# NOAA-GFDL/icebergs

Measured on AMD Instinct MI355X. Metric: berg_steps_per_sec, higher is better.
Workload: dtype f64; 1 GPU; BASELINE configs[4] per-GPU share with configs[1] physics: 10000000 synthetic bergs/GPU (random mass classes), 360x200 lat-lon ocean grid, RK4 drag+Coriolis+melt+mass spreading, dt=1800 s, ignore_traj=T; bergs_per_gpu=10000000, grid=360x200, exchange=none (1 GPU), bergs_alive_at_end=9999583

## Files before the change

### icebergs_amd/csrc/kid_handle.hpp

```cpp
#pragma once
#include "kid_mem.hpp"

struct HipAllocator {
  static constexpr int unknown_error = (int)hipErrorInvalidValue;
  const hipStream_t *stream;
  int alloc(void **p, size_t bytes, kid::MemKind k) const { return (int)(k == kid::MEM_PINNED ? hipHostMalloc(p, bytes) : hipMalloc(p, bytes)); }
  int release(void *p, kid::MemKind k) const { return (int)(k == kid::MEM_PINNED ? hipHostFree(p) : hipFree(p)); }
  int fill(void *p, int byte, size_t bytes) const { return (int)hipMemsetAsync(p, byte, bytes, *stream); }
  int copy(void *dst, const void *src, size_t bytes) const { return (int)hipMemcpy(dst, src, bytes, hipMemcpyDeviceToDevice); }
};
struct Scratch { void *p = nullptr; size_t bytes = 0; };
struct HipMem : kid::MemOwner<HipAllocator> {
  explicit HipMem(const hipStream_t *stream) : kid::MemOwner<HipAllocator>(HipAllocator{stream}) {}
  template <class T> hipError_t dev(T *&p, size_t count, int fill = kid::MEM_NOFILL, kid::MemKind k = kid::MEM_DEVICE) { void *q = nullptr; const int e = alloc(&q, count * sizeof(T), k, fill); p = (T *)q; return (hipError_t)e; }
  template <class T> hipError_t pinned(T *&p, size_t count) { return dev(p, count, kid::MEM_NOFILL, kid::MEM_PINNED); }
  template <class T> hipError_t drop(T *&p) { void *q = p; const int e = release(&q); p = (T *)q; return (hipError_t)e; }
  template <class T> hipError_t regrow(T *&p, size_t keep_count, size_t count) { void *q = p; const int e = grow(&q, keep_count * sizeof(T), count * sizeof(T)); p = (T *)q; return (hipError_t)e; }
  hipError_t reserve(Scratch &t, size_t bytes) {
    if (t.p && t.bytes >= bytes) return hipSuccess;
    int e = release(&t.p);
    if (!e) e = alloc(&t.p, bytes, kid::MEM_DEVICE);
    t.bytes = e ? 0 : bytes;
    return (hipError_t)e;
  }
};

namespace {
enum { KID_PERM_MAX = KID_NB_F64 + KID_NB_I32 + 2 };
struct PermTable { const void *src[KID_PERM_MAX]; void *dst[KID_PERM_MAX]; int n8, n4; };
}

struct ForcingSet { VelRec *vel = nullptr; TrcRec *trc = nullptr; double *pkt = nullptr; DevGrid *d_grid = nullptr; };
struct ForcingState {
  bool have_static = false, have_forcing = false;
  bool have_centres = false;
  bool have_planes = false;
  bool held[KID_NFORCING] = {};
};

struct kid_handle {
  int device = 0;
  hipStream_t own_stream = nullptr, stream = nullptr;
  HipMem mem{&stream}, rp_mem{&stream};
  kid_grid_desc gd{};
  kid_params params{};
  int ni = 0, nj = 0;
  size_t ncell = 0;
  int64_t capacity = 0, n = 0;
  double auto_growth = 0.; int64_t auto_min_free = 0, auto_max_capacity = 0;
  double *d_static[KID_NGRID_STATIC] = {}, *d_forcing[KID_NFORCING] = {};
  GeoRec *d_geo = nullptr; double *d_hotok = nullptr; double *d_latref = nullptr;
  double *d_acc_own = nullptr, *d_acc = nullptr;
  double *d_out = nullptr;
  double *d_totals = nullptr;
  BergPtrs bp{};
  BergPtrs *d_bp = nullptr;
  kid_params *d_params = nullptr;
  bool tables_dirty = true;
  Scratch scan_tmp;
  unsigned long long *d_count = nullptr;
  int *d_redo_list = nullptr;
  hipStream_t side_stream = nullptr; bool pipelined = false;
  int *d_redo_list2 = nullptr, *d_redo_count2 = nullptr;
  int *d_redo_cnt[2][2] = {{nullptr, nullptr}, {nullptr, nullptr}};
  int redo_parity = 0; bool redo_prezeroed = false, acc_prezeroed = false;
  kid::ZeroState zs;
  unsigned long long hot_zero_mask = 0ull;
  bool tail_valid = false;
  bool mig_mode = false;
  int32_t *d_keep = nullptr;
  long long mig_last[2] = {0, 0};
  long long halo_last[2] = {0, 0};
  bool halo_rows_live = false;
  bool env_ever_stored = false;
  bool env_off_requested = false;
  double *d_orient = nullptr;
  hipEvent_t evF[2] = {nullptr, nullptr}, evG[2] = {nullptr, nullptr}; bool evG_live[2] = {false, false};
  int side_mode = 0; int *d_lane = nullptr, *d_lane_alt = nullptr; hipEvent_t evR = nullptr; int lane_step = 1; bool lanes_active = false, carry_valid = false, evC_live = false;
  hipEvent_t evC = nullptr, evP = nullptr;
  ForcingSet fset[2]; int forc_parity = 0;
  struct DebugOpts { bool stable_resort = false, no_plain_build = false, fl_unfused = false, new_order_unfused = false, mts_always_label = false, mts_no_fused = false, rebin_eager = false, chksum_timing = false, no_zero_skip = false;
                     int mts_fused_blocks_cap = 0, mts_poll_limit = 0; } dbg;
  int32_t *d_iceberg_counter = nullptr;
  bool fl_place_warm = false;
  unsigned fl_step = 0;
  int *d_fl_cursor = nullptr;
  int *d_fl_promoted = nullptr;
  int32_t *d_fl_head = nullptr, *d_fl_next = nullptr; int64_t *d_fl_newid = nullptr; long long fl_ev_capacity = 0;
  unsigned *d_key[2] = {nullptr, nullptr}, *d_idx[2] = {nullptr, nullptr};
  Scratch sort_tmp;
  BergPtrs bp_alt{};
  bool rebin_pending = false;
  int64_t rebin_fused_count = 0;
  struct RebinPlan { PermTable t{}; int moved_f[KID_NB_F64] = {}; int nmf = 0; unsigned long long moved = 0ull, zero_skipped = 0ull; const unsigned *perm = nullptr; long long n = 0; } rplan;
  RebinTab *d_rb = nullptr;
  unsigned *d_cell_hist = nullptr; Scratch cscan_tmp; bool stable_resort = false;
  int resort_interval = 16, steps_since_sort = 0;
  MtsDev mts{}; MtsDev *d_mts = nullptr;
  int mb = 0; bool mts_ready = false, mts_dirty = true, have_bonds = false, visited = false;
  unsigned long long *d_key64[2] = {nullptr, nullptr}; int *d_rows[2] = {nullptr, nullptr};
  int *d_static_rows = nullptr; long long static_rows_n = -1, static_rows_cap = 0;
  unsigned long long *d_last_key = nullptr; int *d_order_flag = nullptr; long long order_n = -1;
  unsigned long long *d_bond_sig = nullptr; bool labels_stale = true;
  MtsDev mts_shadow{}; bool mts_shadow_valid = false;
  int conglom_batch = 8;
  Scratch mts_tmp;
  unsigned long long *d_bond_words = nullptr;
  double bond_ext[2] = {0., 0.}; bool bond_ext_valid = false;
  hipGraphExec_t sub_graph_exec = nullptr;
  long long sub_graph_n = -1; int sub_graph_steps = 0; bool sub_graph_pair = false; double sub_graph_dt = 0.; hipStream_t sub_graph_stream = nullptr;
  bool use_graph = true;
  int fused_blocks[2] = {0, 0};
  bool fused_ran = false;
  Flags flags{0, 0, 1, 0, 0};
  bool traj_on = false; kid_traj_params traj_params{}; double *d_traj_f[64] = {}; double *d_traj_day = nullptr; int64_t *d_traj_id = nullptr;
  int32_t *d_traj_year = nullptr, *d_traj_nbonds = nullptr; unsigned long long *d_traj_cursor = nullptr; long long traj_capacity = 0, traj_count_bound = 0; int traj_nf = 0;
  double *d_mig_buf = nullptr; long long mig_capacity = 0; unsigned long long *mig_word = nullptr;
  double *halo_buf = nullptr; long long halo_capacity = 0;
  double *d_btraj_f[16] = {}; int64_t *d_btraj_id[2] = {}; int32_t *d_btraj_i[2] = {}; long long btraj_capacity = 0, btraj_count_bound = 0;
  double *d_spread_mass_old = nullptr;
  double *d_spread_mass_old_own = nullptr;
  ForcingState forc;
  int restart_locate = 0;
  double *d_calv_state = nullptr, *d_calv_scal = nullptr, *d_calv_part = nullptr; unsigned char *d_calv_flag = nullptr; int2 *d_calv_list = nullptr; double *calv_host = nullptr; kid_calving_params calv_params{};
  bool calving_on = false, calving_first_call = true, rmean_init = false, rmean_hflx_init = false;
  double *d_ingest_stage = nullptr; size_t ingest_stage_count = 0; unsigned long long *d_ingest_key = nullptr;
  bool profile = false;
  hipEvent_t ev0 = nullptr, ev1 = nullptr, ev2 = nullptr, ev3 = nullptr;
  std::vector<std::pair<hipEvent_t, hipEvent_t>> pending;
  double berg_ms = 0., all_ms = 0.; int64_t berg_launches = 0;
  bool repro = false;
  struct Repro { double *stage = nullptr; int32_t *key = nullptr; unsigned long long *mask = nullptr; int *srows = nullptr; long long srows_n = -1;
                 unsigned long long *k64[2] = {nullptr, nullptr}; int *rows[2] = {nullptr, nullptr}; unsigned *k32[2] = {nullptr, nullptr};
                 int *cs = nullptr; double *cell_heat = nullptr, *part = nullptr; Scratch tmp; } rp;
  double *d_budget = nullptr, *d_budget_plane = nullptr;
  std::string err;
};

#define KID_HIP(h, call)                                                                      \
  do {                                                                                        \
    hipError_t e__ = (call);                                                                  \
    if (e__ != hipSuccess) {                                                                  \
      (h)->err = std::string(#call) + ": " + hipGetErrorString(e__);                          \
      return KID_EHIP;                                                                        \
    }                                                                                         \
  } while (0)

extern "C" {
static int refresh_tables(kid_handle *h), join_side(kid_handle *h);
static int rebin_flush(kid_handle *h);
static int rebin_plan(kid_handle *h, bool dead_last);
static int rebin_core(kid_handle *h, bool with_lane, int *list, const int *list_count), rebin_apply(kid_handle *h, bool with_lane, int *list, const int *list_count);
static bool plain_namelist(const kid_handle *h), lanes_eligible(const kid_handle *h);
static int repro_refuse(kid_handle *h);
static int mts_check_timeout(kid_handle *h), mts_fold_scalars(kid_handle *h);
static int halo_bergs_supported(kid_handle *h, const char *what);
static int auto_reserve(kid_handle *h, int64_t need, const char *what);
}
```

### icebergs_amd/csrc/kid_hip.hip

```cpp
#include <algorithm>
#include <chrono>
#include <cmath>
#include <cstdio>
#include <cstdlib>
#include <cstring>
#include <string.h>
#include <string>
#include <type_traits>
#include <utility>
#include <vector>
#include <unordered_map>
#include <hip/hip_runtime.h>
#include <rocprim/rocprim.hpp>
#include "../../include/kid.h"
#include "kid_device.hpp"
#include "kid_thermo.hpp"
#include "kid_footloose.hpp"
#include "kid_berg_kernel.hpp"
#include "kid_rows_plan.hpp"
#include "kid_fl_contact.hpp"
#include "kid_reserve_plan.hpp"

using namespace kid;

#ifdef KID_HOT_PLAIN_SEPARATE
namespace kid { void launch_hot_plain(bool store_env, bool rebin, unsigned nblocks, void *stream, const DevGrid *gtab, const kid_params *pp, const void *bp, long long n,
                                      double *acc, size_t ncell, const void *flags, const void *redo); }
#else
#include "kid_hot_plain.inc"
#endif

namespace {

__global__ void __launch_bounds__(256) footloose_kernel(const DevGrid g, const kid_params *__restrict__ pp, const BergPtrs *__restrict__ bt,
                                                        const FlChildCtx cx, double *__restrict__ acc, const size_t ncell) {
  const long long q = (long long)blockIdx.x * 256ll + threadIdx.x;
  if (q >= cx.n) return;
  const BergPtrs &b = *bt;
  if (b.i[KID_BI_ALIVE][q] == 0) return;
  footloose_one(g, *pp, b, cx, q, acc, ncell, acc - KID_NSCALAR);
}

__global__ void set_berg_table_kernel(const BergPtrs src, BergPtrs *dst) { if (threadIdx.x == 0 && blockIdx.x == 0) *dst = src; }
__global__ void set_rebin_table_kernel(const RebinTab src, RebinTab *dst) { if (threadIdx.x == 0 && blockIdx.x == 0) *dst = src; }
__global__ void set_params_kernel(const kid_params src, kid_params *dst) { if (threadIdx.x == 0 && blockIdx.x == 0) *dst = src; }
__global__ void set_time_kernel(int32_t year, double yearday, kid_params *dst) { if (threadIdx.x == 0 && blockIdx.x == 0) { dst->current_year = year; dst->current_yearday = yearday; } }

#include "kid_mts.inc"
#include "kid_fl_interact.inc"

}

#include "kid_handle.hpp"

static int halo_rows_refuse(kid_handle *h, const char *what) {
  if (!h->halo_rows_live) return KID_OK;
  h->err = std::string(what) + ": halo rows are resident (copies of the neighbours' bergs, kid_unpack_immigrants); the next kid_evolve_icebergs retires them";
  return KID_EINVAL;
}
#include "kid_cells.inc"

static int check_params(kid_handle *h, const kid_params *p) {
  if (p->dem && !p->mts) { h->err = "dem needs mts=T (the DEM forces live on the MTS sub-steps)"; return KID_EINVAL; }
  if (p->mts) {
    if (p->Runge_not_Verlet) { h->err = "Runge_not_Verlet must be false to use MTS or DEM (FW:1485-1490)"; return KID_EINVAL; }
    if (p->old_interp_flds_order) { h->err = "old_interp_flds_order is false whenever mts/dem is on (FW:1483)"; return KID_EINVAL; }
    if (p->mts_sub_steps < 1) { h->err = "mts_sub_steps must be >= 1 (pass the value ice_bergs_framework_init derives, FW:1296-1301)"; return KID_EINVAL; }
    if (p->dem && !p->explicit_inner_mts) { h->err = "dem forces explicit_inner_mts=T (FW:1433)"; return KID_EINVAL; }
    if (p->dem && !p->iceberg_bonds_on) { h->err = "dem needs iceberg_bonds_on"; return KID_EINVAL; }
    if (p->max_bonds < 1 || p->max_bonds > KID_MAX_BONDS) { h->err = "max_bonds out of range"; return KID_EINVAL; }
    if (p->use_broken_bonds_for_substep_contact && !(p->break_bonds_on_sub_steps && p->dem && p->iceberg_bonds_on)) {
      h->err = "use_broken_bonds_for_substep_contact requires break_bonds_on_sub_steps, dem and iceberg_bonds_on (FW:1438-1447)"; return KID_EINVAL; }
    if (p->footloose) { h->err = "footloose together with mts is not implemented"; return KID_EUNSUPPORTED; }
  } else if (p->interactive_icebergs_on || p->iceberg_bonds_on) {
    if (p->Runge_not_Verlet) { h->err = "interacting / bonded bergs under the single-time-step scheme are implemented for Verlet only (Runge_not_Verlet=F)"; return KID_EUNSUPPORTED; }
    if (p->footloose && p->iceberg_bonds_on) { h->err = "footloose together with iceberg_bonds_on: bonded footloose calving (edge elements that calve, IB:2566-2585) is not implemented"; return KID_EUNSUPPORTED; }
    if (p->iceberg_bonds_on && !p->interactive_icebergs_on) { h->err = "iceberg_bonds_on without interactive_icebergs_on is not implemented"; return KID_EUNSUPPORTED; }
    if (p->max_bonds < 1 || p->max_bonds > KID_MAX_BONDS) { h->err = "max_bonds out of range"; return KID_EINVAL; }
  }
  if (p->tidal_drift > 0.) { h->err = "tidal_drift needs FMS's random stream: not supported"; return KID_EUNSUPPORTED; }
  if (p->find_melt_using_spread_mass && (p->mts || p->interactive_icebergs_on || p->footloose)) {
    h->err = "find_melt_using_spread_mass is implemented for the plain evolve loop only (no bonds, interactions or footloose)";
    return KID_EUNSUPPORTED;
  }
  if (p->Runge_not_Verlet && p->footloose) { h->err = "Runge_not_Verlet must be false to use footloose (FW:1485-1490)"; return KID_EINVAL; }
  if (p->footloose && !p->use_operator_splitting) { h->err = "use_operator_splitting must be true to use footloose (FW:1476)"; return KID_EINVAL; }
  return KID_OK;
}

extern "C" {

#ifndef KID_BUILD_ID
#define KID_BUILD_ID "unknown"
#endif
const char *kid_version(void) {
  return "kid_hip 0.3 (gfx950) src " KID_BUILD_ID
#ifdef KID_EXACT_MATH
         " exact-math"
#endif
#ifdef KID_EXPERIMENTS
         " EXPERIMENTS"
#endif
      ;
}
int64_t kid_sizeof(int which) {
  switch (which) { case 0: return (int64_t)sizeof(kid_params); case 1: return (int64_t)sizeof(kid_grid_desc);
                   case 2: return (int64_t)sizeof(kid_berg_soa); case 3: return (int64_t)sizeof(kid_bond_soa);
                   case 4: return (int64_t)sizeof(kid_forcing_in);
                   case 5: return (int64_t)sizeof(kid_calving_params); case 6: return (int64_t)sizeof(kid_calving_in); default: return -1; }
}
#ifdef KID_EXP_TIMING
int kid_exp_timing(unsigned long long *out, int reset) {
  if (out) {
    std::vector<unsigned long long> all((size_t)KID_TPROF_WAVES * 16);
    if (hipMemcpyFromSymbol(all.data(), HIP_SYMBOL(kid_tprof), all.size() * sizeof(unsigned long long)) != hipSuccess) return KID_EHIP;
    for (int q = 0; q < 16; ++q) out[q] = 0ull;
    for (size_t r = 0; r < (size_t)KID_TPROF_WAVES; ++r) for (int q = 0; q < 16; ++q) out[q] += all[r * 16 + q];
  }
  if (reset) {
    void *sym = nullptr;
    if (hipGetSymbolAddress(&sym, HIP_SYMBOL(kid_tprof)) != hipSuccess || hipMemset(sym, 0, (size_t)KID_TPROF_WAVES * 16 * sizeof(unsigned long long)) != hipSuccess) return KID_EHIP;
  }
  return KID_OK;
}
#endif
static thread_local std::string destroy_err;
const char *kid_last_error(const kid_handle *h) { return h ? h->err.c_str() : destroy_err.empty() ? "null handle" : destroy_err.c_str(); }

int kid_create(const kid_grid_desc *grid, const kid_params *params, int64_t capacity, int device, kid_handle **out) {
  if (!grid || !params || !out || capacity <= 0) return KID_EINVAL;
  if (capacity > (int64_t(1) << 29)) return KID_EINVAL;
  int ndev = 0;
  if (hipGetDeviceCount(&ndev) != hipSuccess || ndev <= 0) return KID_ENODEV;
  if (device < 0 || device >= ndev) return KID_ENODEV;
  kid_handle *h = new kid_handle();
  *out = h;
  h->device = device;
  KID_HIP(h, hipSetDevice(device));
  h->gd = *grid;
  h->ni = grid->ied - grid->isd + 1; h->nj = grid->jed - grid->jsd + 1;
  if (h->ni < 5 || h->nj < 5 || grid->isc - grid->isd < 2 || grid->ied - grid->iec < 2 || grid->jsc - grid->jsd < 2 || grid->jed - grid->jec < 2) {
    h->err = "grid needs a halo of at least 2 cells"; return KID_EINVAL;
  }
  h->ncell = (size_t)h->ni * (size_t)h->nj;
  int rc = check_params(h, params);
  if (rc) return rc;
  h->params = *params;
  h->flags.footprint = footprint_needed(h->params) ? 1 : 0;
  h->capacity = capacity;
  if (getenv("KID_MTS_NO_GRAPH")) h->use_graph = false;
  h->dbg.stable_resort = getenv("KID_STABLE_RESORT") != nullptr; h->dbg.no_plain_build = getenv("KID_NO_PLAIN_BUILD") != nullptr;
  h->dbg.fl_unfused = getenv("KID_FL_UNFUSED") != nullptr; h->dbg.new_order_unfused = getenv("KID_NEW_ORDER_UNFUSED") != nullptr;
  h->dbg.rebin_eager = getenv("KID_REBIN_EAGER") != nullptr; h->dbg.chksum_timing = getenv("KID_CHKSUM_TIMING") != nullptr;
  h->dbg.no_zero_skip = getenv("KID_NO_ZERO_SKIP") != nullptr;
  h->dbg.mts_always_label = getenv("KID_MTS_ALWAYS_LABEL") != nullptr; h->dbg.mts_no_fused = getenv("KID_MTS_NO_FUSED") != nullptr;
  if (const char *e = getenv("KID_MTS_FUSED_BLOCKS_CAP")) h->dbg.mts_fused_blocks_cap = atoi(e);
  if (const char *e = getenv("KID_MTS_POLL_LIMIT")) h->dbg.mts_poll_limit = atoi(e);
  KID_HIP(h, hipStreamCreateWithFlags(&h->own_stream, hipStreamNonBlocking));
  h->stream = h->own_stream;
  const size_t cap = (size_t)capacity;
  for (auto &plane : h->d_static) KID_HIP(h, h->mem.dev(plane, h->ncell, 0));
  for (auto &plane : h->d_forcing) KID_HIP(h, h->mem.dev(plane, h->ncell, 0));
  for (ForcingSet &fs : h->fset) {
    KID_HIP(h, h->mem.dev(fs.vel, h->ncell)); KID_HIP(h, h->mem.dev(fs.trc, h->ncell)); KID_HIP(h, h->mem.dev(fs.d_grid, 1));
    KID_HIP(h, h->mem.dev(fs.pkt, h->ncell * PK_GSTRIDE, 0));
  }
  KID_HIP(h, h->mem.dev(h->d_geo, h->ncell));
  KID_HIP(h, h->mem.dev(h->d_hotok, h->ncell, 0));
  if (grid->grid_is_latlon) KID_HIP(h, h->mem.dev(h->d_latref, 2 * h->ncell));
  KID_HIP(h, h->mem.dev(h->d_acc_own, (size_t)KID_NACC * h->ncell + KID_NSCALAR, 0));
  h->d_acc = h->d_acc_own + KID_NSCALAR;
  KID_HIP(h, h->mem.dev(h->d_out, (size_t)KID_NOUT * h->ncell, 0));
  KID_HIP(h, h->mem.dev(h->d_totals, KID_NSCALAR, 0));
  for (auto &field : h->bp.f) KID_HIP(h, h->mem.dev(field, cap, 0));
  for (auto &field : h->bp.i) KID_HIP(h, h->mem.dev(field, cap, 0));
  KID_HIP(h, h->mem.dev(h->bp.id, cap, 0));
  KID_HIP(h, h->mem.dev(h->d_bp, 1));
  KID_HIP(h, h->mem.dev(h->d_rb, 1));
  KID_HIP(h, h->mem.dev(h->d_params, 1));
  KID_HIP(h, h->mem.dev(h->d_lane, cap, 0));
  KID_HIP(h, h->mem.dev(h->d_count, 4));
  KID_HIP(h, h->mem.dev(h->d_iceberg_counter, h->ncell, 0));
  KID_HIP(h, h->mem.dev(h->d_fl_cursor, 1));
  for (int **q : {&h->d_redo_list, &h->d_redo_list2}) KID_HIP(h, h->mem.dev(*q, cap));
  KID_HIP(h, h->mem.dev(h->d_redo_count2, 4, 0));
  for (int part = 0; part < 2; ++part) for (int par = 0; par < 2; ++par) h->d_redo_cnt[part][par] = h->d_redo_count2 + (2 * part + par);
  for (hipEvent_t *e : {&h->evC, &h->evP, &h->evF[0], &h->evF[1], &h->evG[0], &h->evG[1]}) KID_HIP(h, hipEventCreateWithFlags(e, hipEventDisableTiming));
  for (hipEvent_t *e : {&h->ev0, &h->ev1, &h->ev2, &h->ev3}) KID_HIP(h, hipEventCreate(e));
  KID_HIP(h, hipStreamSynchronize(h->stream));
  return KID_OK;
}

int kid_destroy(kid_handle *h) {
  if (!h) return KID_EINVAL;
  (void)hipSetDevice(h->device);
  (void)hipDeviceSynchronize();
  if (h->sub_graph_exec) (void)hipGraphExecDestroy(h->sub_graph_exec);
  for (hipEvent_t e : {h->evR, h->evC, h->evP, h->evF[0], h->evF[1], h->evG[0], h->evG[1], h->ev0, h->ev1, h->ev2, h->ev3}) if (e) (void)hipEventDestroy(e);
  for (auto &pe : h->pending) { (void)hipEventDestroy(pe.first); (void)hipEventDestroy(pe.second); }
  if (h->own_stream) (void)hipStreamDestroy(h->own_stream);
  const int e_rp = h->rp_mem.free_all(), e_mem = h->mem.free_all();
  const hipError_t e = (hipError_t)(e_rp ? e_rp : e_mem);
  delete h;
  if (e == hipSuccess) return KID_OK;
  destroy_err = std::string("kid_destroy: freeing the handle's memory: ") + hipGetErrorString(e);
  return KID_EHIP;
}

int kid_memory_in_use(int64_t *device_bytes, int64_t *pinned_bytes) {
  if (device_bytes) *device_bytes = kid::mem_in_use(kid::MEM_DEVICE).load();
  if (pinned_bytes) *pinned_bytes = kid::mem_in_use(kid::MEM_PINNED).load();
  return KID_OK;
}

int kid_set_params(kid_handle *h, const kid_params *params) {
  if (!h || !params) return KID_EINVAL;
  int rc = check_params(h, params);
  if (rc) return rc;
  if (!h->tables_dirty && h->d_params) {
    kid_params a = h->params, b = *params;
    a.current_year = b.current_year = 0; a.current_yearday = b.current_yearday = 0.;
    if (std::memcmp(&a, &b, sizeof(kid_params)) == 0) {
      h->params = *params;
      KID_HIP(h, hipSetDevice(h->device));
      hipLaunchKernelGGL(set_time_kernel, dim3(1), dim3(64), 0, h->stream, params->current_year, params->current_yearday, h->d_params);
      KID_HIP(h, hipGetLastError());
      return KID_OK;
    }
  }
  h->params = *params;
  h->tables_dirty = true;
  h->labels_stale = true;
  h->flags.footprint = footprint_needed(h->params) ? 1 : 0;
  if (!h->params.old_interp_flds_order && !h->env_off_requested) h->flags.store_env = 1;
  return KID_OK;
}
static int join_side(kid_handle *h) {
  for (int q = 0; q < 2; ++q)
    if (h->evG_live[q]) { KID_HIP(h, hipStreamWaitEvent(h->stream, h->evG[q], 0)); }
  if (h->evC_live) { KID_HIP(h, hipStreamWaitEvent(h->stream, h->evC, 0)); }
  return KID_OK;
}
static int lanes_drain(kid_handle *h) {
  const int rc = join_side(h);
  if (rc || !h->lanes_active) return rc;
  KID_HIP(h, hipMemsetAsync(h->d_lane, 0, (size_t)h->capacity * sizeof(int), h->stream));
  if (h->d_lane_alt) KID_HIP(h, hipMemsetAsync(h->d_lane_alt, 0, (size_t)h->capacity * sizeof(int), h->stream));
  h->lanes_active = false; h->carry_valid = false; h->lane_step = 1;
  return KID_OK;
}
int kid_set_side_stream(kid_handle *h, void *s, int enable) {
  if (!h) return KID_EINVAL;
  KID_HIP(h, hipSetDevice(h->device));
  int rc = join_side(h);
  if (rc) return rc;
  KID_HIP(h, hipStreamSynchronize(h->stream));
  { const int rc_d = lanes_drain(h); if (rc_d) return rc_d; }
  { const int rc_f = rebin_flush(h); if (rc_f) return rc_f; }
  KID_HIP(h, hipStreamSynchronize(h->stream));
  h->evG_live[0] = h->evG_live[1] = false; h->evC_live = false;
  h->side_stream = (hipStream_t)s;
  h->pipelined = enable == 1;
  h->side_mode = (s && enable == 2) ? 2 : 0;
  return KID_OK;
}
int kid_set_stream(kid_handle *h, void *s) {
  if (!h) return KID_EINVAL;
  h->stream = (hipStream_t)s;
  return KID_OK;
}
static inline int id_iNg(const kid_grid_desc &d) { return d.gni > 0 ? d.gni : d.iec - d.isc + 1; }
static inline int id_ij0(const kid_grid_desc &d) { return d.gni > 0 ? d.gi0 + d.gni * d.gj0 : 0; }
int kid_sync(kid_handle *h) {
  if (!h) return KID_EINVAL;
  KID_HIP(h, hipSetDevice(h->device));
  { const int rc_j = join_side(h); if (rc_j) return rc_j; }
  KID_HIP(h, hipStreamSynchronize(h->stream));
  return mts_check_timeout(h);
}

#include "kid_ingest.inc"
}
#include "kid_rows.inc"
extern "C" {

int kid_upload_bergs(kid_handle *h, const kid_berg_soa *host) {
  if (!h || !host || host->n < 0) return KID_EINVAL;
  if (host->n > h->capacity) { const int rc = auto_reserve(h, host->n, "kid_upload_bergs"); if (rc) return rc; }
  if (host->n > h->capacity) { h->err = "more bergs than capacity"; return KID_ECAPACITY; }
  { const int rc = rows_enter(h, ROWS_CHANGE); if (rc) return rc; }
  const size_t n = (size_t)host->n;
  for (int f = 0; f < KID_NB_F64; ++f) {
    if (host->f64[f]) KID_HIP(h, hipMemcpyAsync(h->bp.f[f], host->f64[f], n * sizeof(double), hipMemcpyHostToDevice, h->stream));
    else KID_HIP(h, hipMemsetAsync(h->bp.f[f], 0, n * sizeof(double), h->stream));
  }
  for (int f = 0; f < KID_NB_I32; ++f) {
    if (host->i32[f]) KID_HIP(h, hipMemcpyAsync(h->bp.i[f], host->i32[f], n * sizeof(int32_t), hipMemcpyHostToDevice, h->stream));
    else if (f == KID_BI_ALIVE) { if (n) hipLaunchKernelGGL(fill_i32_kernel, dim3((unsigned)((n + 255) / 256)), dim3(256), 0, h->stream, h->bp.i[f], 1, (long long)n); }
    else KID_HIP(h, hipMemsetAsync(h->bp.i[f], 0, n * sizeof(int32_t), h->stream));
  }
  if (host->id) KID_HIP(h, hipMemcpyAsync(h->bp.id, host->id, n * sizeof(int64_t), hipMemcpyHostToDevice, h->stream));
  else KID_HIP(h, hipMemsetAsync(h->bp.id, 0, n * sizeof(int64_t), h->stream));
  if (host->i32[KID_BI_INE] && host->i32[KID_BI_JNE]) {
    for (size_t k = 0; k < n; ++k) {
      const int i = host->i32[KID_BI_INE][k], j = host->i32[KID_BI_JNE][k];
      if (i < h->gd.isc - 1 || i > h->gd.iec + 1 || j < h->gd.jsc - 1 || j > h->gd.jec + 1) {
        h->err = "berg cell index (ine,jne) outside the computational domain"; return KID_EINVAL;
      }
    }
  } else if (n > 0) { h->err = "ine/jne are required"; return KID_EINVAL; }
  if (h->bp.orient) { h->bp.orient = nullptr; h->tables_dirty = true; }
  rows_replaced(h, host);
  h->visited = false; h->have_bonds = false;
  KID_HIP(h, hipStreamSynchronize(h->stream));
  return KID_OK;
}

int kid_download_bergs(kid_handle *h, kid_berg_soa *host) {
  if (!h || !host) return KID_EINVAL;
  if (host->n < h->n) { h->err = "host SoA too small"; return KID_EINVAL; }
  { const int rc = rows_enter(h, ROWS_READ); if (rc) return rc; }
  const size_t n = (size_t)h->n;
  for (int f = 0; f < KID_NB_F64; ++f)
    if (host->f64[f]) KID_HIP(h, hipMemcpyAsync(host->f64[f], h->bp.f[f], n * sizeof(double), hipMemcpyDeviceToHost, h->stream));
  for (int f = 0; f < KID_NB_I32; ++f)
    if (host->i32[f]) KID_HIP(h, hipMemcpyAsync(host->i32[f], h->bp.i[f], n * sizeof(int32_t), hipMemcpyDeviceToHost, h->stream));
  if (host->id) KID_HIP(h, hipMemcpyAsync(host->id, h->bp.id, n * sizeof(int64_t), hipMemcpyDeviceToHost, h->stream));
  KID_HIP(h, hipStreamSynchronize(h->stream));
  host->n = h->n;
  return KID_OK;
}

int kid_set_store_environment(kid_handle *h, int on) {
  if (!h) return KID_EINVAL;
  h->flags.store_env = on ? 1 : 0;
  h->env_off_requested = !on;
  return KID_OK;
}

static int refresh_tables(kid_handle *h) {
  if (h->tables_dirty) {
    const int rc = join_side(h);
    if (rc) return rc;
    hipLaunchKernelGGL(set_berg_table_kernel, dim3(1), dim3(64), 0, h->stream, h->bp, h->d_bp);
    hipLaunchKernelGGL(set_params_kernel, dim3(1), dim3(64), 0, h->stream, h->params, h->d_params);
    for (int par = 0; par < 2; ++par) hipLaunchKernelGGL(set_grid_kernel, dim3(1), dim3(64), 0, h->stream, dev_grid(h, par), h->fset[par].d_grid);
    KID_HIP(h, hipGetLastError());
    h->tables_dirty = false;
  }
  return KID_OK;
}
static int fl_place_children(kid_handle *h, long long n_old, int m, unsigned step) {
  if (!h->fl_place_warm) {
    h->fl_place_warm = true;
    hipLaunchKernelGGL(fl_place_children_kernel<BergPtrs>, dim3(1), dim3(64), 0, h->stream, dev_grid(h), (const kid_params *)h->d_params, (const BergPtrs *)h->d_bp, n_old, 0, step);
    KID_HIP(h, hipGetLastError());
  }
  if (m <= 0) return KID_OK;
  hipLaunchKernelGGL(fl_place_children_kernel<BergPtrs>, dim3((unsigned)((m + 63) / 64)), dim3(64), 0, h->stream, dev_grid(h), (const kid_params *)h->d_params, (const BergPtrs *)h->d_bp, n_old, m, step);
  KID_HIP(h, hipGetLastError());
  return KID_OK;
}
static int fl_assign_ids(kid_handle *h, long long n_old, int m) {
  if (m <= 0) return KID_OK;
  if (!h->d_fl_head) KID_HIP(h, h->mem.dev(h->d_fl_head, h->ncell, 0xff));
  if (m > h->fl_ev_capacity) {
    KID_HIP(h, h->mem.drop(h->d_fl_next));
    KID_HIP(h, h->mem.drop(h->d_fl_newid));
    h->fl_ev_capacity = std::max<long long>(2ll * m, 4096);
    KID_HIP(h, h->mem.dev(h->d_fl_next, (size_t)h->fl_ev_capacity));
    KID_HIP(h, h->mem.dev(h->d_fl_newid, (size_t)h->fl_ev_capacity));
  }
  const FlIdCtx x{h->d_fl_head, h->d_fl_next, h->d_fl_newid, h->d_iceberg_counter, n_old, m, id_iNg(h->gd), id_ij0(h->gd)};
  const dim3 grid((unsigned)((m + 255) / 256)), block(256);
  const DevGrid g = dev_grid(h);
  hipLaunchKernelGGL(fl_assign_ids_push<BergPtrs>, grid, block, 0, h->stream, g, (const BergPtrs *)h->d_bp, x);
  hipLaunchKernelGGL(fl_assign_ids_rank<BergPtrs>, grid, block, 0, h->stream, g, (const BergPtrs *)h->d_bp, x);
  hipLaunchKernelGGL(fl_assign_ids_store<BergPtrs>, grid, block, 0, h->stream, g, (const BergPtrs *)h->d_bp, x);
  KID_HIP(h, hipGetLastError());
  return KID_OK;
}
static const char *const fl_full = "footloose calving ran out of capacity: create the handle with room for child bergs";
int kid_footloose_calving(kid_handle *h) {
  if (!h) return KID_EINVAL;
  { const int rc_h = halo_rows_refuse(h, "kid_footloose_calving"); if (rc_h) return rc_h; }
  if (!h->params.footloose || h->n == 0) return KID_OK;
  KID_HIP(h, hipSetDevice(h->device));
  int rc = repro_refuse(h);
  if (rc) return rc;
  rc = rebin_flush(h);
  if (rc) return rc;
  rc = refresh_tables(h);
  if (rc) return rc;
  h->flags.has_fl = 1;
  h->zs.launched_other();
  rc = auto_reserve(h, h->n + h->auto_min_free, "kid_footloose_calving");
  if (rc) return rc;
  KID_HIP(h, hipMemsetAsync(h->d_fl_cursor, 0, sizeof(int), h->stream));
  const unsigned fl_step_now = h->fl_step;
  FlChildCtx cx{h->d_fl_cursor, h->d_iceberg_counter, (long long)h->n, (long long)h->capacity, h->gd.iec - h->gd.isc + 1, h->fl_step++};
  hipLaunchKernelGGL(footloose_kernel, dim3((unsigned)((h->n + 255) / 256)), dim3(256), 0, h->stream, dev_grid(h), h->d_params, h->d_bp, cx, h->d_acc, h->ncell);
  KID_HIP(h, hipGetLastError());
  int appended = 0;
  KID_HIP(h, hipMemcpyAsync(&appended, h->d_fl_cursor, sizeof(int), hipMemcpyDeviceToHost, h->stream));
  KID_HIP(h, hipStreamSynchronize(h->stream));
  if (appended <= h->capacity - h->n) {
    rc = fl_place_children(h, h->n, appended, fl_step_now);
    if (!rc) rc = fl_assign_ids(h, h->n, appended);
    if (rc) return rc;
  }
  return rows_appended(h, appended, nullptr, fl_full);
}
double kid_footloose_uniform(int32_t seed, int64_t berg_id, int64_t step, int32_t draw) {
  return kid_fl_uniform((uint32_t)seed, berg_id, (uint32_t)step, (uint32_t)draw);
}
int kid_set_footloose_step(kid_handle *h, int64_t step) {
  if (!h || step < 0) return KID_EINVAL;
  h->fl_step = (unsigned)step;
  return KID_OK;
}
int kid_get_footloose_step(kid_handle *h, int64_t *step) {
  if (!h || !step) return KID_EINVAL;
  *step = (int64_t)h->fl_step;
  return KID_OK;
}
int kid_set_iceberg_counter(kid_handle *h, const int32_t *counter) {
  if (!h || !counter) return KID_EINVAL;
  KID_HIP(h, hipSetDevice(h->device));
  KID_HIP(h, hipMemcpy(h->d_iceberg_counter, counter, h->ncell * sizeof(int32_t), hipMemcpyHostToDevice));
  return KID_OK;
}
int kid_get_iceberg_counter(kid_handle *h, int32_t *counter) {
  if (!h || !counter) return KID_EINVAL;
  KID_HIP(h, hipSetDevice(h->device));
  KID_HIP(h, hipStreamSynchronize(h->stream));
  KID_HIP(h, hipMemcpy(counter, h->d_iceberg_counter, h->ncell * sizeof(int32_t), hipMemcpyDeviceToHost));
  return KID_OK;
}

#include "kid_mts_host.inc"
#include "kid_calving.inc"
#include "kid_repro.inc"
}
#include "kid_bond_init.inc"
#include "kid_budget.inc"
#include "kid_launch.inc"
#include "kid_reserve.inc"
extern "C" {

int kid_last_redo_count(kid_handle *h, int64_t *count) {
  if (!h || !count) return KID_EINVAL;
  KID_HIP(h, hipSetDevice(h->device));
  { const int rc_j = join_side(h); if (rc_j) return rc_j; }
  int c[4] = {0, 0, 0, 0};
  KID_HIP(h, hipMemcpyAsync(c, h->d_redo_count2, 4 * sizeof(int), hipMemcpyDeviceToHost, h->stream));
  KID_HIP(h, hipStreamSynchronize(h->stream));
  *count = (int64_t)c[0 + h->redo_parity] + (h->pipelined ? (int64_t)c[2 + h->redo_parity] : 0);
  return KID_OK;
}
int kid_rebin_fused_count(kid_handle *h, int64_t *count) {
  if (!h || !count) return KID_EINVAL;
  *count = h->rebin_fused_count;
  return KID_OK;
}
int kid_hot_zero_mask(kid_handle *h, uint64_t *mask) {
  if (!h || !mask) return KID_EINVAL;
  *mask = (uint64_t)h->hot_zero_mask;
  return KID_OK;
}
int kid_profile_enable(kid_handle *h, int on) {
  if (!h) return KID_EINVAL;
  h->profile = on != 0;
  h->berg_ms = 0.; h->all_ms = 0.; h->berg_launches = 0;
  return KID_OK;
}
int kid_profile_get(kid_handle *h, double *berg_ms, int64_t *launches, double *all_ms) {
  if (!h) return KID_EINVAL;
  KID_HIP(h, hipSetDevice(h->device));
  KID_HIP(h, hipStreamSynchronize(h->stream));
  for (auto &pe : h->pending) {
    float ms = 0.f;
    KID_HIP(h, hipEventElapsedTime(&ms, pe.first, pe.second));
    h->berg_ms += ms;
    (void)hipEventDestroy(pe.first); (void)hipEventDestroy(pe.second);
  }
  h->pending.clear();
  if (berg_ms) *berg_ms = h->berg_ms;
  if (launches) *launches = h->berg_launches;
  if (all_ms) *all_ms = h->all_ms;
  return KID_OK;
}

}

#include "kid_locate.inc"
#include "kid_restart.inc"
#include "kid_traj.inc"
#include "kid_migrate.inc"
#include "kid_halo_bergs.inc"
#include "kid_halo.inc"
#include "kid_chksum.inc"
#include "kid_chksum_device.inc"
```

### icebergs_amd/csrc/kid_launch.inc

```

static bool plain_namelist(const kid_handle *h) {
  const kid_params &p = h->params;
  bool same = true;
#define KID_X(name, plain, flp) same = same && (p.name == (decltype(p.name))(plain));
  KID_SWITCHES(KID_X)
#undef KID_X
  const Flags &f = h->flags;
  return same && h->gd.grid_is_latlon && !p.pass_fields_to_ocean_model && !f.has_static && !f.has_fl && !f.footprint && !f.no_diag &&
         !h->dbg.no_plain_build;
}
static bool fl_profile_namelist(const kid_handle *h) {
  const kid_params &p = h->params;
  bool same = true;
#define KID_X(name, plain, flp) same = same && (p.name == (decltype(p.name))(flp));
  KID_SWITCHES(KID_X)
#undef KID_X
  const Flags &f = h->flags;
  return same && !h->gd.grid_is_latlon && !p.pass_fields_to_ocean_model && !f.has_static && f.has_fl && !f.footprint && !f.no_diag && !h->dbg.no_plain_build;
}
static bool lanes_eligible(const kid_handle *h) {
  const kid_params &p = h->params;
  return kid::lanes_eligible(h->side_mode, h->side_stream != nullptr, h->repro, p.static_icebergs != 0, p.mts != 0, p.interactive_icebergs_on != 0,
                             p.footloose != 0, p.grounding_fraction, p.find_melt_using_spread_mass != 0, (long long)h->n);
}

struct BergLaunch { const DevGrid *gtab; bool plain, flprof; };
static BergLaunch berg_launch(const kid_handle *h) { return {h->fset[h->forc_parity].d_grid, plain_namelist(h), fl_profile_namelist(h)}; }

template <bool RK, bool OLD, unsigned PH, bool FAST, int K, bool STAGE>
static int launch_instance(kid_handle *h, const BergLaunch &c, hipStream_t s, unsigned nblocks, const Redo &redo) {
  static_assert(instance_exists(OLD, PH, STAGE), "no call site requests this instance (kid_launch_select.hpp)");
  hipLaunchKernelGGL((berg_kernel<RK, OLD, PH, FAST, K, STAGE>), dim3(nblocks), dim3(FAST ? KID_HOT_WG : 64), 0, s, c.gtab, h->d_params, h->d_bp, (long long)h->n, h->d_acc, h->ncell, h->flags, redo);
  KID_HIP(h, hipGetLastError());
  return KID_OK;
}
template <bool RK, bool OLD, unsigned PH, bool STAGE>
static int launch_hot(kid_handle *h, const BergLaunch &c, hipStream_t s, const Redo &redo, bool rebin = false) {
  const unsigned nbp = (unsigned)((redo.klen + KID_HOT_WG - 1) / KID_HOT_WG);
  const int k = hot_build_k(RK, OLD, PH, c.plain, c.flprof, h->flags.store_env != 0, STAGE);
  h->hot_zero_mask = 0ull;
  if constexpr (hot_build_k(RK, OLD, PH, true, false, false, STAGE) == 1) {
    if (k == 1 || k == 3) {
      Redo plain = redo;
      plain.zero = h->hot_zero_mask = known_zero_mask(h);
      kid::launch_hot_plain(k == 3, rebin, nbp, (void *)s, c.gtab, h->d_params, h->d_bp, (long long)h->n, h->d_acc, h->ncell, &h->flags, &plain);
      KID_HIP(h, hipGetLastError());
      return KID_OK;
    }
  }
  if constexpr (hot_build_k(RK, OLD, PH, false, true, false, STAGE) == 2) {
    if (k == 2 && !rebin) return launch_instance<RK, OLD, PH, true, 2, STAGE>(h, c, s, nbp, redo);
  }
  if (rebin || k != 0) { h->err = "no such hot build of the per-berg kernel"; return KID_EINVAL; }
  return launch_instance<RK, OLD, PH, true, 0, STAGE>(h, c, s, nbp, redo);
}
template <bool RK, bool OLD, unsigned PH, bool STAGE>
static int launch_general(kid_handle *h, const BergLaunch &c, hipStream_t s, const Redo &redo, long long rows) {
  return launch_instance<RK, OLD, PH, false, 0, STAGE>(h, c, s, (unsigned)std::min<long long>((rows + 63) / 64, 2048), redo);
}
template <unsigned PH, class F>
static int with_instance(kid_handle *h, bool stage, F &&f) {
  const bool rk = h->params.Runge_not_Verlet != 0, old = h->params.old_interp_flds_order != 0;
  auto go = [&](auto RK, auto OLD, auto STAGE) -> int {
    if constexpr (instance_exists(decltype(OLD)::value, PH, decltype(STAGE)::value)) return f(RK, OLD, STAGE);
    else { h->err = "no per-berg kernel for this phase mask, interpolation order and summation mode"; return KID_EINVAL; }
  };
  auto order = [&](auto RK, auto STAGE) { return old ? go(RK, std::true_type{}, STAGE) : go(RK, std::false_type{}, STAGE); };
  auto integrator = [&](auto STAGE) { return rk ? order(std::true_type{}, STAGE) : order(std::false_type{}, STAGE); };
  return stage ? integrator(std::true_type{}) : integrator(std::false_type{});
}

static int wait_general_builds(kid_handle *h, int part, int nparts) {
  if (h->evG_live[part]) KID_HIP(h, hipStreamWaitEvent(h->stream, h->evG[part], 0));
  if (nparts == 1 && h->evG_live[1]) KID_HIP(h, hipStreamWaitEvent(h->stream, h->evG[1], 0));
  return KID_OK;
}
static int zero_redo_counter(kid_handle *h, int *count) {
  if (!h->redo_prezeroed) KID_HIP(h, hipMemsetAsync(count, 0, sizeof(int), h->stream));
  return KID_OK;
}
struct ProfilePair { hipEvent_t e0 = nullptr, e1 = nullptr; };
static int profile_start(kid_handle *h, ProfilePair &t) {
  if (!h->profile) return KID_OK;
  KID_HIP(h, hipEventCreate(&t.e0)); KID_HIP(h, hipEventCreate(&t.e1));
  KID_HIP(h, hipEventRecord(t.e0, h->stream));
  return KID_OK;
}
static int profile_stop(kid_handle *h, const ProfilePair &t) {
  if (!h->profile) return KID_OK;
  KID_HIP(h, hipEventRecord(t.e1, h->stream));
  h->pending.emplace_back(t.e0, t.e1); h->berg_launches++;
  return KID_OK;
}
template <unsigned PH>
static int rebin_take_or_flush(kid_handle *h, bool whole, RebinTab &rtab, bool &fused) {
  fused = false;
  if (!h->rebin_pending) return KID_OK;
  fused = PH == PH_STEP && rebin_fusable(h) && whole && h->rplan.n == h->n && (h->rplan.zero_skipped & ~known_zero_mask(h)) == 0ull &&
          rebin_table(h, h->flags.store_env ? 3 : 1, rtab);
  return fused ? KID_OK : rebin_flush(h);
}
static int rebin_bind(kid_handle *h, const RebinTab &rtab, Redo &redo) {
  hipLaunchKernelGGL(set_rebin_table_kernel, dim3(1), dim3(64), 0, h->stream, rtab, h->d_rb);
  KID_HIP(h, hipGetLastError());
  redo.rb = h->d_rb; redo.perm = h->rplan.perm;
  return KID_OK;
}
static int rebin_hand_over(kid_handle *h, Redo &redo) {
  h->rebin_pending = false; redo.rb = nullptr; redo.perm = nullptr; h->rebin_fused_count++;
  return rebin_swap(h);
}
template <bool RK, bool OLD, unsigned PH>
static int launch_general_part(kid_handle *h, const BergLaunch &c, const Redo &redo, int part, int nparts) {
  hipStream_t gs = (nparts == 2) ? h->side_stream : h->stream;
  if (nparts == 2) { KID_HIP(h, hipEventRecord(h->evF[part], h->stream)); KID_HIP(h, hipStreamWaitEvent(gs, h->evF[part], 0)); }
  const int rc = launch_general<RK, OLD, PH, false>(h, c, gs, redo, redo.klen);
  if (rc) return rc;
  if (nparts == 2) KID_HIP(h, hipEventRecord(h->evG[part], gs));
  h->evG_live[part] = nparts == 2;
  return KID_OK;
}
template <unsigned PH>
static int launch_berg_part(kid_handle *h, const BergLaunch &c, bool stage, const RebinTab *rtab, Redo redo, int part, int nparts) {
  int rc = KID_OK;
  if (rtab) { rc = rebin_bind(h, *rtab, redo); if (rc) return rc; }
  rc = wait_general_builds(h, part, nparts);
  if (!rc) rc = zero_redo_counter(h, redo.count);
  ProfilePair t;
  if (!rc) rc = profile_start(h, t);
  if (rc) return rc;
  return with_instance<PH>(h, stage, [&](auto RK, auto OLD, auto STAGE) -> int {
    constexpr bool rk = decltype(RK)::value, old = decltype(OLD)::value;
    int r = launch_hot<rk, old, PH, decltype(STAGE)::value>(h, c, h->stream, redo, rtab != nullptr);
    if constexpr (decltype(STAGE)::value) {
      if (!r) r = launch_general<rk, old, PH, true>(h, c, h->stream, redo, redo.klen);
      if (!r) r = profile_stop(h, t);
      h->evG_live[part] = false;
      return r;
    } else {
      if (!r) r = profile_stop(h, t);
      if (!r && rtab) r = rebin_hand_over(h, redo);
      return r ? r : launch_general_part<rk, old, PH>(h, c, redo, part, nparts);
    }
  });
}
template <unsigned PH>
static int launch_phase(kid_handle *h, long long range_k0 = 0, long long range_len = -1) {
  if (need_forcing(h)) return KID_EINVAL;
  if (h->n == 0 || range_len == 0) return KID_OK;
  const bool old = h->params.old_interp_flds_order != 0, whole = range_k0 == 0 && range_len < 0;
  if (!old && !(PH & PH_INTERP) && (PH & (PH_EVOLVE | PH_THERMO)) && !h->flags.store_env) {
    h->err = "this entry point reads the bergs' stored environment, which kid_set_store_environment has switched off (use kid_run_step, or switch it on)";
    return KID_EINVAL;
  }
  h->zs.launched_berg((PH & PH_EVOLVE) != 0, (PH & PH_THERMO) != 0, h->params.Runge_not_Verlet != 0, h->params.bergy_bit_erosion_fraction == 0.,
                      h->flags.has_fl != 0, (PH & PH_FL) != 0);
  int rc = repro_refuse(h);
  if (!rc) rc = lanes_drain(h);
  RebinTab rtab;
  bool rebin_fused = false;
  if (!rc) rc = rebin_take_or_flush<PH>(h, whole, rtab, rebin_fused);
  if (!rc) rc = refresh_tables(h);
  if (rc) return rc;
  const BergLaunch c = berg_launch(h);
  rows_killed(h);
  if (h->flags.store_env || !old) h->env_ever_stored = true;
  const bool stage = (PH & PH_SCATTER) != 0 && h->repro;
  const int nparts = launch_parts(h->pipelined, stage, h->params.mts != 0, h->params.footloose != 0, (long long)h->n, range_len < 0);
  const long long half = ((h->n / 2 + 255) / 256) * 256;
  for (int part = 0; part < nparts && !rc; ++part) {
    const long long k0 = (nparts == 1) ? range_k0 : (part == 0 ? 0 : half);
    const long long klen = (nparts == 1) ? (range_len < 0 ? h->n : range_len) : (part == 0 ? half : h->n - half);
    const Redo redo{part == 0 ? h->d_redo_list : h->d_redo_list2, h->d_redo_cnt[part][h->redo_parity], k0, klen, nullptr, 0,
                    h->d_fl_cursor, h->d_iceberg_counter, (long long)h->capacity, h->gd.iec - h->gd.isc + 1, h->fl_step,
                    StageTab{h->rp.stage, h->rp.key, h->rp.mask, (long long)h->capacity}};
    rc = launch_berg_part<PH>(h, c, stage, rebin_fused ? &rtab : nullptr, redo, part, nparts);
  }
  if (nparts == 1) h->evG_live[1] = false;
  h->redo_prezeroed = false;
  if (rc) return rc;
  if (stage) return repro_fold(h, (PH & PH_THERMO) != 0, (PH & (PH_SPREAD | PH_TSPREAD)) != 0, range_k0, range_len < 0 ? h->n : range_len);
  return KID_OK;
}
template <unsigned PH>
static int launch_berg(kid_handle *h, long long range_k0 = 0, long long range_len = -1) {
  static_assert(instance_exists(true, PH, false) && instance_exists(false, PH, false), "this mask is bound to one order: launch_ordered");
  return launch_phase<PH>(h, range_k0, range_len);
}
template <unsigned X>
static int launch_ordered(kid_handle *h, long long range_k0 = 0, long long range_len = -1) {
  static_assert(!(X & PH_INTERP) && instance_exists(true, X, false) && instance_exists(false, PH_INTERP | X, false), "not an (old, new) pair of masks");
  return h->params.old_interp_flds_order ? launch_phase<X>(h, range_k0, range_len) : launch_phase<PH_INTERP | X>(h, range_k0, range_len);
}

template <bool OLDV>
static int launch_berg_lanes(kid_handle *h) {
  constexpr unsigned PH = OLDV ? PH_STEP : (PH_INTERP | PH_STEP);
  static_assert(instance_exists(OLDV, PH, false), "the fused step of this order");
  if (need_forcing(h)) return KID_EINVAL;
  { const int rc_f = rebin_flush(h); if (rc_f) return rc_f; }
  { int rc_t = refresh_tables(h); if (rc_t) return rc_t; }
  const BergLaunch c = berg_launch(h);
  h->zs.launched_berg(true, true, h->params.Runge_not_Verlet != 0, h->params.bergy_bit_erosion_fraction == 0., h->flags.has_fl != 0, false);
  hipStream_t M = h->stream, S = h->side_stream;
  const int s = h->lane_step, par = s & 1;
  rows_killed(h);
  if (h->flags.store_env || !OLDV) h->env_ever_stored = true;
  h->lanes_active = true;
  for (int q = 0; q < 2; ++q) if (h->evG_live[q] && h->pipelined) { KID_HIP(h, hipStreamWaitEvent(M, h->evG[q], 0)); h->evG_live[q] = false; }
  if (!h->redo_prezeroed) {
    if (h->evC_live) KID_HIP(h, hipStreamWaitEvent(M, h->evC, 0));
    KID_HIP(h, hipMemsetAsync(h->d_redo_cnt[0][par], 0, sizeof(int), M));
  }
  int *list_new = par ? h->d_redo_list2 : h->d_redo_list, *list_old = par ? h->d_redo_list : h->d_redo_list2;
  const Redo hot{list_new, h->d_redo_cnt[0][par], 0, h->n, h->d_lane, s};
  const Redo carry{list_old, h->d_redo_cnt[0][par ^ 1], 0, h->n, nullptr, 0};
  ProfilePair t;
  if (h->profile) { KID_HIP(h, hipEventCreate(&t.e0)); KID_HIP(h, hipEventCreate(&t.e1)); }
  hipEvent_t evP = h->profile ? t.e0 : h->evP, evF = h->profile ? t.e1 : h->evF[0];
  KID_HIP(h, hipEventRecord(evP, M));
  KID_HIP(h, hipStreamWaitEvent(S, evP, 0));
  const bool rebin_now = h->resort_interval > 0 && ++h->steps_since_sort >= h->resort_interval && !h->have_bonds && !h->dbg.stable_resort;
  int rebin_rc = KID_OK;
  auto lanes = [&](auto RK) -> int {
    constexpr bool rk = decltype(RK)::value;
    if (h->carry_valid) { const int r = launch_general<rk, OLDV, PH, false>(h, c, S, carry, h->n); if (r) return r; }
    KID_HIP(h, hipEventRecord(h->evC, S)); h->evC_live = true;
    { const int r = launch_hot<rk, OLDV, PH, false>(h, c, M, hot); if (r) return r; }
    KID_HIP(h, hipEventRecord(evF, M));
    if (h->profile) { h->pending.emplace_back(t.e0, t.e1); h->berg_launches++; }
    if (rebin_now) {
      KID_HIP(h, hipStreamWaitEvent(M, h->evC, 0));
      rebin_rc = rebin_core(h, true, list_new, h->d_redo_cnt[0][par]);
      if (!h->evR) KID_HIP(h, hipEventCreateWithFlags(&h->evR, hipEventDisableTiming));
      KID_HIP(h, hipEventRecord(h->evR, M)); KID_HIP(h, hipStreamWaitEvent(S, h->evR, 0));
    } else KID_HIP(h, hipStreamWaitEvent(S, evF, 0));
    { const int r = launch_general<rk, OLDV, PH, false>(h, c, S, hot, h->n); if (r) return r; }
    KID_HIP(h, hipEventRecord(h->evG[0], S)); h->evG_live[0] = true;
    return KID_OK;
  };
  const int rc = h->params.Runge_not_Verlet ? lanes(std::true_type{}) : lanes(std::false_type{});
  if (rc || rebin_rc) return rc ? rc : rebin_rc;
  if (rebin_now) h->steps_since_sort = 0;
  h->carry_valid = true;
  h->lane_step = s + 1;
  h->redo_prezeroed = false;
  return KID_OK;
}

static int launch_fused_step(kid_handle *h) {
  if (!lanes_eligible(h)) return launch_ordered<PH_STEP>(h);
  return h->params.old_interp_flds_order ? launch_berg_lanes<true>(h) : launch_berg_lanes<false>(h);
}

static int step_mts(kid_handle *h) {
  int rc = h->visited ? KID_OK : mts_first_visit(h);
  if (!rc && !h->params.static_icebergs) rc = kid_evolve_icebergs_mts(h);
  if (!rc) rc = kid_interp_gridded_fields_to_bergs(h);
  if (!rc) rc = kid_set_conglom_ids(h);
  if (!rc) rc = bond_orientations(h);
  return rc ? rc : launch_berg<PH_THERMO | PH_SPREAD>(h);
}
static int step_interactive(kid_handle *h) {
  const kid_params &p = h->params;
  const bool contact = (p.contact_distance > 0.) || (p.contact_spring_coef != p.spring_coef);
  int rc = h->visited ? KID_OK : sts_ia_first_visit(h);
  if (!rc && !p.old_interp_flds_order) rc = launch_berg<PH_INTERP>(h);
  if (!rc && !p.static_icebergs) rc = kid_evolve_icebergs_interactive(h);
  if (!rc && p.footloose) rc = kid_footloose_calving(h);
  if (!rc && contact) rc = kid_set_conglom_ids(h);
  if (!rc) rc = bond_orientations(h);
  if (!rc && p.footloose) rc = kid_adjust_fl_berg_interactivity(h, nullptr);
  return rc ? rc : launch_ordered<PH_THERMO | PH_SPREAD>(h);
}
static int step_footloose_fused(kid_handle *h) {
  { const int rc_a = auto_reserve(h, h->n + h->auto_min_free, "kid_step_local"); if (rc_a) return rc_a; }
  h->flags.has_fl = 1;
  KID_HIP(h, hipMemsetAsync(h->d_fl_cursor, 0, sizeof(int), h->stream));
  const long long n_old = h->n;
  int rc = launch_ordered<PH_STEP_FL>(h);
  const unsigned fl_step_now = h->fl_step;
  h->fl_step += 1u;
  if (rc) return rc;
  int appended = 0;
  KID_HIP(h, hipMemcpyAsync(&appended, h->d_fl_cursor, sizeof(int), hipMemcpyDeviceToHost, h->stream));
  KID_HIP(h, hipStreamSynchronize(h->stream));
  if (appended <= h->capacity - n_old) {
    rc = fl_place_children(h, n_old, appended, fl_step_now);
    if (!rc) rc = fl_assign_ids(h, n_old, appended);
    if (rc) return rc;
  }
  rc = rows_appended(h, appended, nullptr, fl_full);
  return rc ? rc : launch_ordered<PH_THERMO | PH_SPREAD>(h, n_old, appended);
}
static int step_footloose_phases(kid_handle *h) {
  int rc = h->params.static_icebergs ? launch_berg<PH_INTERP>(h) : launch_berg<PH_INTERP | PH_EVOLVE>(h);
  if (!rc) rc = kid_footloose_calving(h);
  return rc ? rc : launch_berg<PH_INTERP | PH_THERMO | PH_SPREAD>(h);
}
static int step_spread_mass(kid_handle *h) {
  const kid_params &p = h->params;
  if (!h->d_spread_mass_old) {
    KID_HIP(h, h->mem.dev(h->d_spread_mass_old_own, 2 * h->ncell, 0));
    h->d_spread_mass_old = h->d_spread_mass_old_own;
  }
  int rc = KID_OK;
  if (!p.static_icebergs) { rc = p.old_interp_flds_order ? launch_berg<PH_EVOLVE>(h) : launch_berg<PH_INTERP | PH_EVOLVE>(h); if (rc) return rc; }
  rc = zero_planes(h, ON_OCEAN_ALL);
  if (rc) return rc;
  const Flags keep = h->flags;
  h->flags.no_diag = 1; h->flags.footprint = 0;
  rc = launch_berg<PH_SPREAD>(h);
  h->flags = keep;
  if (!rc) rc = gather_mass_and_reset(h, h->d_spread_mass_old);
  if (rc) return rc;
  if (!p.Iceberg_melt_without_decay) return launch_ordered<PH_THERMO | PH_SPREAD>(h);
  rc = launch_ordered<PH_THERMO | PH_TSPREAD>(h);
  if (!rc) rc = gather_mass_and_reset(h, h->d_spread_mass_old + h->ncell);
  return rc ? rc : launch_berg<PH_SPREAD>(h);
}
static int step_default(kid_handle *h) {
  const kid_params &p = h->params;
  const bool old = p.old_interp_flds_order != 0;
  if (!p.static_icebergs && (old || !h->dbg.new_order_unfused || lanes_eligible(h))) return launch_fused_step(h);
  if (old) return launch_berg<PH_THERMO | PH_SPREAD>(h);
  const int rc = p.static_icebergs ? launch_berg<PH_INTERP>(h) : launch_berg<PH_INTERP | PH_EVOLVE>(h);
  return rc ? rc : launch_berg<PH_INTERP | PH_THERMO | PH_SPREAD>(h);
}

extern "C" {

int kid_interp_gridded_fields_to_bergs(kid_handle *h) {
  if (!h) return KID_EINVAL;
  { const int rc_h = halo_rows_refuse(h, "kid_interp_gridded_fields_to_bergs"); if (rc_h) return rc_h; }
  KID_HIP(h, hipSetDevice(h->device));
  int rc = launch_berg<PH_INTERP>(h);
  if (rc || !h->params.mts) return rc;
  return mts_depth(h);
}
int kid_evolve_icebergs(kid_handle *h) {
  if (!h) return KID_EINVAL;
  KID_HIP(h, hipSetDevice(h->device));
  if (h->params.static_icebergs) return KID_OK;
  { const int rc_r = repro_refuse(h); if (rc_r) return rc_r; }
  if (h->params.mts) return kid_evolve_icebergs_mts(h);
  if (h->params.interactive_icebergs_on) return kid_evolve_icebergs_interactive(h);
  return launch_berg<PH_EVOLVE>(h);
}
int kid_thermodynamics(kid_handle *h) {
  if (!h) return KID_EINVAL;
  { const int rc_h = halo_rows_refuse(h, "kid_thermodynamics"); if (rc_h) return rc_h; }
  KID_HIP(h, hipSetDevice(h->device));
  if (h->params.find_melt_using_spread_mass && (!h->d_spread_mass_old || h->d_spread_mass_old == h->d_spread_mass_old_own)) {
    h->err = "find_melt_using_spread_mass: the phase entry points do not gather spread_mass_old (IB:5490-5503); use kid_run_step / kid_step_local";
    return KID_EUNSUPPORTED;
  }
  const int rc = zero_planes(h, ON_OCEAN_VEL);
  return rc ? rc : launch_berg<PH_THERMO>(h);
}
int kid_create_gridded_icebergs_fields(kid_handle *h) {
  if (!h) return KID_EINVAL;
  { const int rc_h = halo_rows_refuse(h, "kid_create_gridded_icebergs_fields"); if (rc_h) return rc_h; }
  KID_HIP(h, hipSetDevice(h->device));
  int rc = zero_planes(h, ON_OCEAN_ALL);
  if (!rc) rc = launch_berg<PH_SPREAD>(h);
  return rc ? rc : launch_gather(h);
}

int kid_step_local(kid_handle *h) {
  if (!h) return KID_EINVAL;
  { const int rc_h = halo_rows_refuse(h, "kid_step_local"); if (rc_h) return rc_h; }
  KID_HIP(h, hipSetDevice(h->device));
  int rc = h->acc_prezeroed ? KID_OK : kid_zero_accumulators(h);
  h->acc_prezeroed = false;
  if (!rc) rc = repro_refuse(h);
  if (!rc && h->rebin_pending && !rebin_fusable(h)) rc = rebin_flush(h);
  if (rc) return rc;
  const kid_params &p = h->params;
  if (p.mts) return step_mts(h);
  if (p.interactive_icebergs_on) return step_interactive(h);
  if (p.footloose) return (!p.static_icebergs && !h->dbg.fl_unfused) ? step_footloose_fused(h) : step_footloose_phases(h);
  if (p.find_melt_using_spread_mass) return step_spread_mass(h);
  return step_default(h);
}
int kid_step_gather(kid_handle *h) {
  if (!h) return KID_EINVAL;
  { const int rc_h = halo_rows_refuse(h, "kid_step_gather"); if (rc_h) return rc_h; }
  KID_HIP(h, hipSetDevice(h->device));
  return launch_gather(h);
}
int kid_run_step(kid_handle *h, int nsteps) {
  if (!h || nsteps < 0) return KID_EINVAL;
  for (int s = 0; s < nsteps; ++s) {
    int rc = kid_step_local(h);
    if (rc) return rc;
    rc = kid_step_gather(h);
    if (rc) return rc;
    if (!h->lanes_active && !h->params.mts && !h->params.interactive_icebergs_on && h->resort_interval > 0 && ++h->steps_since_sort >= h->resort_interval) {
      rc = kid_move_berg_between_cells(h);
      if (rc) return rc;
    }
  }
  return KID_OK;
}

}
```

### icebergs_amd/csrc/kid_reserve.inc

```

namespace {
struct ReserveOps {
  kid_handle *h;
  HipMem &owner(int o) const { return o ? h->rp_mem : h->mem; }
  int alloc(int o, void **p, size_t bytes, int fill) const { return owner(o).alloc(p, bytes, kid::MEM_DEVICE, fill); }
  int release(int o, void **p) const {
    if (!*p) return 0;
    const int e = (int)hipStreamSynchronize(h->stream);
    const int e2 = owner(o).release(p);
    return e ? e : e2;
  }
  int copy(void *dst, const void *src, size_t bytes) const { return (int)hipMemcpyAsync(dst, src, bytes, hipMemcpyDeviceToDevice, h->stream); }
  int move_down(void *dst, const void *src, size_t bytes) const {
    if ((const char *)dst + bytes <= (const char *)src) return copy(dst, src, bytes);
    std::vector<char> tmp(bytes);
    int e = (int)hipStreamSynchronize(h->stream);
    if (!e) e = (int)hipMemcpy(tmp.data(), src, bytes, hipMemcpyDeviceToHost);
    if (!e) e = (int)hipMemcpy(dst, tmp.data(), bytes, hipMemcpyHostToDevice);
    return e;
  }
  int fill(void *p, int byte, size_t bytes) const { return (int)hipMemsetAsync(p, byte, bytes, h->stream); }
};

struct ReserveList {
  struct Back { void (*put)(void *member, void *v); void *member; };
  std::vector<kid::ReserveBlock> blocks;
  std::vector<void *> value;
  std::vector<Back> back;
  template <class T>
  void add(T *&p, int kind, int fill = kid::RESERVE_NOFILL, size_t slots = 1, int owner = 0, size_t fixed_bytes = 0, size_t *bytes = nullptr, size_t elem = sizeof(T)) {
    if (!p) return;
    blocks.push_back(kid::ReserveBlock{nullptr, bytes, kind, owner, fill, elem, slots, fixed_bytes});
    value.push_back((void *)p);
    back.push_back(Back{[](void *member, void *v) { *static_cast<T **>(member) = static_cast<T *>(v); }, (void *)&p});
  }
  void add(Scratch &t, int kind, int owner = 0, size_t fixed_bytes = 0) {
    if (!t.p) return;
    blocks.push_back(kid::ReserveBlock{nullptr, &t.bytes, kind, owner, kid::RESERVE_NOFILL, 1, 1, fixed_bytes ? fixed_bytes : 1});
    value.push_back(t.p);
    back.push_back(Back{[](void *member, void *v) { *static_cast<void **>(member) = v; }, (void *)&t.p});
  }
  void bind() { for (size_t q = 0; q < blocks.size(); ++q) blocks[q].member = &value[q]; }
  void store() { for (size_t q = 0; q < blocks.size(); ++q) back[q].put(back[q].member, value[q]); }
};
}

extern "C" {

static int reserve_list(kid_handle *h, int64_t new_cap, ReserveList &L) {
  using namespace kid;
  const size_t cap = (size_t)new_cap;
  for (auto &field : h->bp.f) L.add(field, RESERVE_STATE, 0);
  for (auto &field : h->bp.i) L.add(field, RESERVE_STATE, 0);
  L.add(h->bp.id, RESERVE_STATE, 0);
  if (h->mts_ready) {
    const size_t mbs = (size_t)(h->mb > 0 ? h->mb : 1);
    L.add(h->mts.bcount, RESERVE_STATE, 0);
    L.add(h->mts.bother_id, RESERVE_STATE, 0, mbs);
    L.add(h->mts.bbroken, RESERVE_STATE, 0, mbs);
    L.add(h->mts.bother_row, RESERVE_STATE, 0xff, mbs);
    L.add(h->mts.bother_slot, RESERVE_STATE, 0xff, mbs);
    for (auto &field : h->mts.bf) L.add(field, RESERVE_STATE, 0, mbs);
    for (int32_t **q : {&h->mts.rank, &h->mts.order, &h->mts.label}) L.add(*q, RESERVE_STATE);
    L.add(h->d_last_key, RESERVE_STATE);
    L.add(h->d_bond_sig, RESERVE_STATE, 0);
  }
  L.add(h->d_orient, RESERVE_STATE);
  L.add(h->d_lane, RESERVE_REALLOC, 0);
  L.add(h->d_redo_list, RESERVE_REALLOC);
  L.add(h->d_redo_list2, RESERVE_REALLOC);
  if (h->mts_ready) {
    for (int32_t **q : {&h->mts.root_flag, &h->mts.root_scan}) L.add(*q, RESERVE_REALLOC);
    L.add(h->mts.rec, RESERVE_REALLOC, 0, 3 * 8);
    for (int q = 0; q < 2; ++q) { L.add(h->d_key64[q], RESERVE_REALLOC); L.add(h->d_rows[q], RESERVE_REALLOC); }
    size_t b1 = 0, b2 = 0;
    KID_HIP(h, rocprim::radix_sort_pairs(nullptr, b1, h->d_key64[0], h->d_key64[1], h->d_rows[0], h->d_rows[1], cap, 0, 64, h->stream));
    KID_HIP(h, rocprim::exclusive_scan(nullptr, b2, h->mts.root_flag, h->mts.root_scan, 0, cap, rocprim::plus<int>(), h->stream));
    L.add(h->mts_tmp, RESERVE_REALLOC, 0, std::max(b1, b2));
  }
  if (h->rp.stage) {
    L.add(h->rp.stage, RESERVE_REALLOC, RESERVE_NOFILL, (size_t)KID_ST_N, 1);
    L.add(h->rp.key, RESERVE_REALLOC, RESERVE_NOFILL, 1, 1);
    L.add(h->rp.mask, RESERVE_REALLOC, RESERVE_NOFILL, 1, 1);
    L.add(h->rp.srows, RESERVE_REALLOC, RESERVE_NOFILL, 1, 1);
    for (int q = 0; q < 2; ++q) {
      L.add(h->rp.k64[q], RESERVE_REALLOC, RESERVE_NOFILL, 1, 1); L.add(h->rp.rows[q], RESERVE_REALLOC, RESERVE_NOFILL, 1, 1); L.add(h->rp.k32[q], RESERVE_REALLOC, RESERVE_NOFILL, 1, 1);
    }
    size_t b64 = 0, b32 = 0;
    KID_HIP(h, rocprim::radix_sort_pairs(nullptr, b64, h->rp.k64[0], h->rp.k64[1], h->rp.rows[0], h->rp.rows[1], cap, 0, 64, h->stream));
    KID_HIP(h, rocprim::radix_sort_pairs(nullptr, b32, h->rp.k32[0], h->rp.k32[1], h->rp.rows[0], h->rp.rows[1], cap, 0, 32, h->stream));
    L.add(h->rp.tmp, RESERVE_REALLOC, 1, std::max(b64, b32));
  }
  for (auto &field : h->bp_alt.f) L.add(field, RESERVE_LAZY);
  for (auto &field : h->bp_alt.i) L.add(field, RESERVE_LAZY);
  L.add(h->bp_alt.id, RESERVE_LAZY);
  for (unsigned **q : {&h->d_key[0], &h->d_key[1], &h->d_idx[0], &h->d_idx[1], &h->d_cell_hist}) L.add(*q, RESERVE_LAZY);
  for (Scratch *t : {&h->sort_tmp, &h->scan_tmp, &h->cscan_tmp}) L.add(*t, RESERVE_LAZY);
  L.add(h->d_lane_alt, RESERVE_LAZY);
  L.add(h->d_keep, RESERVE_LAZY);
  L.add(h->d_static_rows, RESERVE_LAZY);
  L.add(h->d_budget, RESERVE_LAZY);
  L.bind();
  return KID_OK;
}

static int reserve_core(kid_handle *h, int64_t new_cap) {
  const int64_t old_cap = h->capacity;
  ReserveList L;
  { const int rc = reserve_list(h, new_cap, L); if (rc) return rc; }
  ReserveOps ops{h};
  const bool had_orient = h->bp.orient != nullptr;
  const kid::ReserveResult r = kid::reserve_apply(ops, L.blocks.data(), (int)L.blocks.size(), h->n, old_cap, new_cap);
  L.store();
  if (had_orient) h->bp.orient = h->d_orient;
  h->rplan = kid_handle::RebinPlan{};
  h->static_rows_cap = 0;
  rows_orders_stale(h);
  h->order_n = -1; h->labels_stale = true;
  if (h->sub_graph_exec) { (void)hipGraphExecDestroy(h->sub_graph_exec); h->sub_graph_exec = nullptr; h->sub_graph_n = -1; }
  h->tables_dirty = true; h->mts_dirty = true;
  if (r.grown) {
    h->capacity = new_cap;
    if (h->mts_ready) h->mts.stride = (long long)new_cap;
  }
  int rc = h->mts_ready ? mts_refresh(h) : refresh_tables(h);
  if (!rc) { const hipError_t e = hipStreamSynchronize(h->stream); if (e != hipSuccess) { h->err = std::string("kid_reserve: ") + hipGetErrorString(e); rc = KID_EHIP; } }
  if (r.error) {
    h->err = std::string("kid_reserve: ") + hipGetErrorString((hipError_t)r.error) +
             (r.grown ? " while freeing a block of the old capacity (the handle is at the new capacity)"
                      : " while growing from " + std::to_string(old_cap) + " to " + std::to_string(new_cap) + " rows (the handle keeps the old capacity)") +
             (r.restride_failed ? "; the bond tables could not be put back to the old stride and hold nothing usable: upload the bonds again" : "");
    if (r.restride_failed) h->have_bonds = false;
    return KID_EHIP;
  }
  return rc;
}

static int auto_reserve(kid_handle *h, int64_t need, const char *what) {
  if (h->auto_growth == 0. || need <= h->capacity) return KID_OK;
  int64_t next = h->capacity;
  const int rc_n = kid::reserve_next_capacity(h->capacity, need, h->auto_growth, h->auto_max_capacity, &next);
  if (rc_n == kid::RESERVE_ECAPACITY) {
    h->err = std::string(what) + ": " + std::to_string(need) + " rows are needed, more than the max_capacity of kid_set_auto_reserve, " +
             std::to_string(kid::reserve_max_capacity(h->auto_max_capacity)) + "; nothing was written";
    return KID_ECAPACITY;
  }
  if (rc_n) { h->err = std::string(what) + ": auto-reserve was given a count that is no row count"; return KID_EINVAL; }
  { const int rc = rows_enter(h, ROWS_CHANGE); if (rc) return rc; }
  return reserve_core(h, next);
}

int kid_capacity(kid_handle *h, int64_t *rows) {
  if (!h || !rows) return KID_EINVAL;
  *rows = h->capacity;
  return KID_OK;
}

int kid_reserve(kid_handle *h, int64_t rows) {
  if (!h) return KID_EINVAL;
  if (rows > kid::RESERVE_MAX_ROWS) { h->err = "kid_reserve: more than 2^29 rows (the per-berg kernel addresses a row by a 32-bit byte offset)"; return KID_EINVAL; }
  if (rows <= h->capacity) return KID_OK;
  { const int rc = rows_enter(h, ROWS_CHANGE); if (rc) return rc; }
  return reserve_core(h, rows);
}

int kid_set_auto_reserve(kid_handle *h, int64_t min_free, double growth, int64_t max_capacity) {
  if (!h) return KID_EINVAL;
  if (!kid::reserve_policy_valid(min_free, growth, max_capacity)) {
    h->err = "kid_set_auto_reserve: growth is 0 (off) or >= 1, min_free >= 0, max_capacity between 0 (meaning 2^29) and 2^29";
    return KID_EINVAL;
  }
  h->auto_growth = growth;
  h->auto_min_free = growth == 0. ? 0 : min_free;
  h->auto_max_capacity = growth == 0. ? 0 : max_capacity;
  return KID_OK;
}

}
```

### icebergs_amd/csrc/kid_rows.inc

```
namespace {
__device__ __forceinline__ long long wave_reserve(bool mine, unsigned long long *cursor) {
  const unsigned long long m = __ballot(mine);
  if (!m) return -1;
  const int lane = (int)__lane_id();
  unsigned long long base = 0;
  if (lane == 0) base = atomicAdd(cursor, (unsigned long long)__popcll(m));
  base = __shfl(base, 0);
  return mine ? (long long)base + __popcll(m & ((1ull << lane) - 1ull)) : -1;
}
__global__ void __launch_bounds__(256) count_alive_kernel(const int32_t *alive, long long n, unsigned long long *out) {
  __shared__ unsigned wsum[4];
  unsigned local = 0;
  for (long long k = (long long)blockIdx.x * 256ll + threadIdx.x; k < n; k += (long long)gridDim.x * 256ll) local += alive[k] ? 1u : 0u;
#pragma unroll
  for (int d = 32; d >= 1; d >>= 1) local += __shfl_xor(local, d);
  if ((threadIdx.x & 63) == 0) wsum[threadIdx.x >> 6] = local;
  __syncthreads();
  if (threadIdx.x == 0) atomicAdd(out, (unsigned long long)(wsum[0] + wsum[1] + wsum[2] + wsum[3]));
}
__global__ void __launch_bounds__(256) compact_perm_kernel(const int32_t *keep, const unsigned *pos, unsigned *perm, long long n) {
  const long long k = (long long)blockIdx.x * 256ll + threadIdx.x;
  if (k < n && keep[k]) perm[pos[k]] = (unsigned)k;
}
struct KeepSel { int isc, iec, jsc, jec; const double *halo; };
__global__ void __launch_bounds__(256) keep_flags_kernel(const int32_t *alive, const int32_t *ine, const int32_t *jne, const KeepSel s, int32_t *keep, long long n) {
  const long long k = (long long)blockIdx.x * 256ll + threadIdx.x;
  if (k >= n) return;
  const int i = ine[k], j = jne[k];
  const bool waiting = (i < s.isc || i > s.iec || j < s.jsc || j > s.jec) && !(s.halo && s.halo[k] >= 0.5);
  keep[k] = (alive[k] != 0 || waiting) ? 1 : 0;
}
__global__ void __launch_bounds__(256) alive_to_u32_kernel(const int32_t *alive, unsigned *flag, long long n) {
  const long long k = (long long)blockIdx.x * 256ll + threadIdx.x;
  if (k < n) flag[k] = alive[k] ? 1u : 0u;
}
__global__ void __launch_bounds__(256) cell_key_kernel(const int32_t *ine, const int32_t *jne, const int32_t *alive, int isd, int jsd, int ni,
                                                       unsigned dead_key, unsigned *key, unsigned *idx, long long n) {
  const long long k = (long long)blockIdx.x * 256ll + threadIdx.x;
  if (k < n) {
    key[k] = alive[k] ? (unsigned)((ine[k] - isd) + (jne[k] - jsd) * ni) : dead_key;
    idx[k] = (unsigned)k;
  }
}
__global__ void __launch_bounds__(256) cell_rank_kernel(const int32_t *ine, const int32_t *jne, const int32_t *alive, int isd, int jsd, int ni,
                                                        unsigned dead_key, unsigned *key, unsigned *rank, unsigned *hist, long long n) {
  const long long k = (long long)blockIdx.x * 256ll + threadIdx.x;
  const bool in = k < n;
  const unsigned c = in ? (alive[k] ? (unsigned)((ine[k] - isd) + (jne[k] - jsd) * ni) : dead_key) : 0xffffffffu;
  const int lane = (int)__lane_id();
  const unsigned prev = __shfl_up(c, 1);
  const bool head = (lane == 0) || (prev != c);
  const unsigned long long heads = __ballot(head);
  const unsigned long long below = heads & ((lane == 63) ? ~0ull : ((2ull << lane) - 1ull));
  const int head_lane = 63 - __clzll(below);
  const unsigned long long above = (lane == 63) ? 0ull : (heads >> (lane + 1));
  const int next_head = above ? lane + 1 + (__ffsll((long long)above) - 1) : 64;
  unsigned base = 0u;
  if (head && in) base = atomicAdd(hist + c, (unsigned)(next_head - lane));
  base = __shfl(base, head_lane);
  if (in) { key[k] = c; rank[k] = base + (unsigned)(lane - head_lane); }
}
__global__ void __launch_bounds__(256) cell_place_kernel(const unsigned *key, const unsigned *rank, const unsigned *start, unsigned *perm, unsigned *inv, long long n) {
  const long long k = (long long)blockIdx.x * 256ll + threadIdx.x;
  if (k < n) { const unsigned pos = start[key[k]] + rank[k]; perm[pos] = (unsigned)k; inv[k] = pos; }
}
__global__ void __launch_bounds__(256) translate_list_kernel(int *list, const int *count, const unsigned *inv) {
  const int total = *count;
  for (int t = blockIdx.x * 256 + threadIdx.x; t < total; t += gridDim.x * 256) list[t] = (int)inv[list[t]];
}
__global__ void __launch_bounds__(256) translate_rows_kernel(int *rows, const unsigned *inv, long long n) {
  const long long q = (long long)blockIdx.x * 256ll + threadIdx.x;
  if (q < n) rows[q] = (int)inv[rows[q]];
}
__global__ void __launch_bounds__(256) permute_all_kernel(const PermTable t, const unsigned *perm, long long n) {
  const long long k = (long long)blockIdx.x * 256ll + threadIdx.x;
  if (k >= n) return;
  const unsigned p = perm[k];
  int f = 0;
  for (; f + 4 <= t.n8; f += 4) {
    const double a = ((const double *)t.src[f])[p], b = ((const double *)t.src[f + 1])[p], c = ((const double *)t.src[f + 2])[p], d = ((const double *)t.src[f + 3])[p];
    ((double *)t.dst[f])[k] = a; ((double *)t.dst[f + 1])[k] = b; ((double *)t.dst[f + 2])[k] = c; ((double *)t.dst[f + 3])[k] = d;
  }
  for (; f < t.n8; ++f) ((double *)t.dst[f])[k] = ((const double *)t.src[f])[p];
  for (; f < t.n8 + t.n4; ++f) ((int32_t *)t.dst[f])[k] = ((const int32_t *)t.src[f])[p];
}
__global__ void __launch_bounds__(256) fill_i32_kernel(int32_t *p, int32_t v, long long n) {
  const long long k = (long long)blockIdx.x * 256ll + threadIdx.x;
  if (k < n) p[k] = v;
}
}
__global__ void __launch_bounds__(256) halo_berg_count_kernel(const int32_t *alive, const double *halo, long long n, unsigned long long *count) {
  const long long k = (long long)blockIdx.x * 256ll + threadIdx.x;
  const unsigned long long m = __ballot(k < n && alive[k] != 0 && halo[k] >= 0.5);
  if (m && __lane_id() == 0) atomicAdd(count, (unsigned long long)__popcll(m));
}

extern "C" {

static void rows_orders_stale(kid_handle *h) { h->static_rows_n = -1; h->rp.srows_n = -1; }
static void rows_replaced(kid_handle *h, const kid_berg_soa *host) {
  const size_t n = (size_t)host->n;
  bool any_static = false, any_fl = false;
  for (int f = 0; f < KID_NB_F64; ++f) {
    bool nz = false;
    if (host->f64[f]) for (size_t k = 0; k < n && !nz; ++k) nz = host->f64[f][k] != 0. || std::signbit(host->f64[f][k]);
    h->zs.uploaded(f, nz);
    any_static = any_static || (nz && marks_has_static(f)); any_fl = any_fl || (nz && marks_has_fl(f));
  }
  h->flags.has_static = any_static ? 1 : 0;
  h->flags.has_fl = (any_fl || h->params.footloose) ? 1 : 0;
  rows_orders_stale(h);
  h->tail_valid = false; h->env_ever_stored = false; h->halo_rows_live = false;
  h->n = host->n;
}
static void rows_moved(kid_handle *h, bool dead_last) { rows_orders_stale(h); h->tail_valid = dead_last; }
static void rows_truncated(kid_handle *h, int64_t n) { rows_orders_stale(h); h->tail_valid = false; h->n = n; }
static void rows_killed(kid_handle *h) { h->tail_valid = false; }
static void rows_located(kid_handle *h) {
  rows_orders_stale(h);
  rows_killed(h);
  h->zs.uploaded_nonzero[KID_B_XI] = true; h->zs.uploaded_nonzero[KID_B_YJ] = true;
}
static int rows_appended(kid_handle *h, int64_t m, const double *records, const char *full) {
  if (m <= 0) return KID_OK;
  rows_orders_stale(h);
  h->tail_valid = false;
  if (!h->params.old_interp_flds_order) h->env_ever_stored = true;
  if (!records) h->zs.appended_by_kernel();
  else {
    for (int64_t q = 0; q < m; ++q)
      for (int w = 0; w < MIG_WIDTH; ++w) {
        const double word = records[(size_t)q * MIG_WIDTH + w];
        if (WIRE_RECORD[w].kind != WIRE_F64 || (word == 0. && !std::signbit(word))) continue;
        const int f = WIRE_RECORD[w].field;
        h->zs.appended_word(f);
        if (marks_has_static(f)) h->flags.has_static = 1;
        if (marks_has_fl(f)) h->flags.has_fl = 1;
      }
    h->zs.uploaded_nonzero[KID_B_UVEL_OLD] |= h->zs.uploaded_nonzero[KID_B_UVEL]; h->zs.uploaded_nonzero[KID_B_VVEL_OLD] |= h->zs.uploaded_nonzero[KID_B_VVEL];
    h->zs.uploaded_nonzero[KID_B_LON_OLD] |= h->zs.uploaded_nonzero[KID_B_LON]; h->zs.uploaded_nonzero[KID_B_LAT_OLD] |= h->zs.uploaded_nonzero[KID_B_LAT];
  }
  if (m > h->capacity - h->n) {
    h->err = full;
    if (h->auto_growth != 0.) h->err += " (the launch tried to append " + std::to_string(m) + " rows, " + std::to_string(h->capacity - h->n) + " were free: raise min_free of kid_set_auto_reserve)";
    h->n = h->capacity;
    return KID_ECAPACITY;
  }
  h->n += m;
  return KID_OK;
}

enum RowsMode { ROWS_READ, ROWS_CHANGE };
static int rows_enter(kid_handle *h, RowsMode mode) {
  KID_HIP(h, hipSetDevice(h->device));
  const int rc = mode == ROWS_CHANGE ? lanes_drain(h) : join_side(h);
  return rc ? rc : rebin_flush(h);
}
static int count_rows(kid_handle *h, const int32_t *flags, const double *halo, int64_t *count) {
  unsigned long long cnt = 0;
  *count = 0;
  if (h->n == 0) return KID_OK;
  const long long n = h->n;
  KID_HIP(h, hipMemsetAsync(h->d_count, 0, sizeof(cnt), h->stream));
  if (halo) hipLaunchKernelGGL(halo_berg_count_kernel, dim3((unsigned)((n + 255) / 256)), dim3(256), 0, h->stream, flags, halo, n, h->d_count);
  else hipLaunchKernelGGL(count_alive_kernel, dim3((unsigned)std::min<long long>((n + 255) / 256, 1024)), dim3(256), 0, h->stream, flags, n, h->d_count);
  KID_HIP(h, hipGetLastError());
  KID_HIP(h, hipMemcpyAsync(&cnt, h->d_count, sizeof(cnt), hipMemcpyDeviceToHost, h->stream));
  KID_HIP(h, hipStreamSynchronize(h->stream));
  *count = (int64_t)cnt;
  return KID_OK;
}

static int layout_flags(kid_handle *h, const int32_t **flags) {
  *flags = h->bp.i[KID_BI_ALIVE];
  if (!h->mig_mode || h->n == 0) return KID_OK;
  if (!h->d_keep) KID_HIP(h, h->mem.dev(h->d_keep, (size_t)h->capacity));
  const KeepSel ks{h->gd.isc, h->gd.iec, h->gd.jsc, h->gd.jec, h->flags.has_static ? h->bp.f[KID_B_HALO_BERG] : nullptr};
  hipLaunchKernelGGL(keep_flags_kernel, dim3((unsigned)((h->n + 255) / 256)), dim3(256), 0, h->stream, h->bp.i[KID_BI_ALIVE], h->bp.i[KID_BI_INE], h->bp.i[KID_BI_JNE], ks, h->d_keep, (long long)h->n);
  KID_HIP(h, hipGetLastError());
  *flags = h->d_keep;
  return KID_OK;
}

int kid_num_bergs(kid_handle *h, int64_t *n_slots, int64_t *n_alive) {
  if (!h) return KID_EINVAL;
  { const int rc = rows_enter(h, ROWS_READ); if (rc) return rc; }
  if (n_slots) *n_slots = h->n;
  if (n_alive) {
    int64_t cnt = 0;
    { const int rc = count_rows(h, h->bp.i[KID_BI_ALIVE], nullptr, &cnt); if (rc) return rc; }
    *n_alive = cnt;
    if (h->tail_valid && h->mig_mode && cnt < h->n) {
      const int32_t *flags = nullptr;
      { const int rc = layout_flags(h, &flags); if (rc) return rc; }
      { const int rc = count_rows(h, flags, nullptr, &cnt); if (rc) return rc; }
    }
    if (h->tail_valid && cnt < h->n) {
      rows_truncated(h, cnt);
      if (n_slots) *n_slots = h->n;
    }
  }
  return KID_OK;
}

static bool field_never_written(const kid_handle *h, int f) {
  const kid_params &p = h->params;
  return kid::field_never_written(NeverWrittenIn{p.footloose != 0, p.mts != 0, h->calving_on, p.periodic_reentry != 0, p.Runge_not_Verlet != 0,
                                                 h->flags.has_fl != 0, h->env_ever_stored}, f);
}
static unsigned long long known_zero_mask(const kid_handle *h) {
  if (h->dbg.no_zero_skip) return 0ull;
  return kid::known_zero_mask(h->zs, field_never_written(h, KID_B_HEAT_DENSITY), h->params.Runge_not_Verlet != 0, h->params.bergy_bit_erosion_fraction == 0.);
}
static int perm_storage(kid_handle *h) {
  if (h->d_key[0]) return KID_OK;
  h->stable_resort = h->dbg.stable_resort;
  for (unsigned **q : {&h->d_key[0], &h->d_key[1], &h->d_idx[0], &h->d_idx[1]}) KID_HIP(h, h->mem.dev(*q, (size_t)h->capacity));
  size_t tmp = 0;
  KID_HIP(h, rocprim::radix_sort_pairs(nullptr, tmp, h->d_key[0], h->d_key[1], h->d_idx[0], h->d_idx[1], (size_t)h->capacity, 0u, 32u, h->stream));
  KID_HIP(h, h->mem.reserve(h->sort_tmp, tmp));
  KID_HIP(h, h->mem.dev(h->d_cell_hist, (size_t)h->ncell + 1));
  tmp = 0;
  KID_HIP(h, rocprim::exclusive_scan(nullptr, tmp, h->d_cell_hist, h->d_cell_hist, 0u, (size_t)h->ncell + 1, rocprim::plus<unsigned>(), h->stream));
  KID_HIP(h, h->mem.reserve(h->cscan_tmp, tmp));
  tmp = 0;
  KID_HIP(h, rocprim::exclusive_scan(nullptr, tmp, h->d_key[0], h->d_key[1], 0u, (size_t)h->capacity, rocprim::plus<unsigned>(), h->stream));
  KID_HIP(h, h->mem.reserve(h->scan_tmp, tmp));
  for (auto &field : h->bp_alt.f) KID_HIP(h, h->mem.dev(field, (size_t)h->capacity));
  for (auto &field : h->bp_alt.i) KID_HIP(h, h->mem.dev(field, (size_t)h->capacity));
  KID_HIP(h, h->mem.dev(h->bp_alt.id, (size_t)h->capacity));
  return KID_OK;
}
static void perm_fields(kid_handle *h, const unsigned *perm, long long n) {
  kid_handle::RebinPlan &pl = h->rplan;
  pl = kid_handle::RebinPlan{};
  PermTable &t = pl.t;
  const unsigned long long zeros = known_zero_mask(h);
  for (int f = 0; f < KID_NB_F64; ++f) {
    if (!h->zs.uploaded_nonzero[f] && field_never_written(h, f)) continue;
    if ((zeros >> f) & 1ull) { pl.zero_skipped |= 1ull << f; continue; }
    t.src[t.n8] = h->bp.f[f]; t.dst[t.n8] = h->bp_alt.f[f]; ++t.n8; pl.moved_f[pl.nmf++] = f; pl.moved |= 1ull << f;
  }
  t.src[t.n8] = h->bp.id; t.dst[t.n8] = h->bp_alt.id; ++t.n8;
  for (int f = 0; f < KID_NB_I32; ++f) { t.src[t.n8 + t.n4] = h->bp.i[f]; t.dst[t.n8 + t.n4] = h->bp_alt.i[f]; ++t.n4; }
  pl.perm = perm; pl.n = n;
}
static const char *const bonds_keep_rows = "bergs with bonds keep their rows: no re-binning while bond tables exist";

int kid_compact_bergs(kid_handle *h) {
  if (!h) return KID_EINVAL;
  { const int rc = rows_enter(h, ROWS_CHANGE); if (rc) return rc; }
  if (h->n == 0) return KID_OK;
  if (h->have_bonds) { h->err = bonds_keep_rows; return KID_EUNSUPPORTED; }
  { const int rc = perm_storage(h); if (rc) return rc; }
  const long long n = h->n;
  const unsigned nb = (unsigned)((n + 255) / 256);
  const int32_t *live = nullptr;
  { const int rc_l = layout_flags(h, &live); if (rc_l) return rc_l; }
  unsigned *flag = h->d_key[0], *pos = h->d_key[1], *perm = h->d_idx[1];
  hipLaunchKernelGGL(alive_to_u32_kernel, dim3(nb), dim3(256), 0, h->stream, live, flag, n);
  size_t tmp = h->scan_tmp.bytes;
  KID_HIP(h, rocprim::exclusive_scan(h->scan_tmp.p, tmp, flag, pos, 0u, (size_t)n, rocprim::plus<unsigned>(), h->stream));
  hipLaunchKernelGGL(compact_perm_kernel, dim3(nb), dim3(256), 0, h->stream, live, (const unsigned *)pos, perm, n);
  KID_HIP(h, hipGetLastError());
  int64_t kept = 0;
  { const int rc = count_rows(h, live, nullptr, &kept); if (rc) return rc; }
  rows_moved(h, false);
  perm_fields(h, perm, kept);
  { const int rc = rebin_apply(h, false, nullptr, nullptr); if (rc) return rc; }
  rows_truncated(h, kept);
  return KID_OK;
}

static bool rebin_fusable(const kid_handle *h) {
  const kid_params &p = h->params;
  return !h->dbg.rebin_eager && !h->repro && !h->mig_mode && !h->pipelined && h->forc.have_forcing && p.Runge_not_Verlet && p.old_interp_flds_order &&
         !p.static_icebergs && !p.mts && !p.interactive_icebergs_on && !p.footloose && !p.find_melt_using_spread_mass && !lanes_eligible(h) && plain_namelist(h);
}
int kid_move_berg_between_cells(kid_handle *h) {
  if (!h) return KID_EINVAL;
  { const int rc_h = halo_rows_refuse(h, "kid_move_berg_between_cells"); if (rc_h) return rc_h; }
  { const int rc_e = rows_enter(h, ROWS_CHANGE); if (rc_e) return rc_e; }
  h->steps_since_sort = 0;
  if (h->n == 0) return KID_OK;
  if (h->have_bonds) { h->err = bonds_keep_rows; return KID_EUNSUPPORTED; }
  int rc = rebin_plan(h, true);
  if (rc) return rc;
  if (rebin_fusable(h)) h->rebin_pending = true;
  else { rc = rebin_apply(h, false, nullptr, nullptr); if (rc) return rc; }
  return KID_OK;
}
static int rebin_core(kid_handle *h, bool with_lane, int *list, const int *list_count) {
  const int rc = rebin_plan(h, false);
  return rc ? rc : rebin_apply(h, with_lane, list, list_count);
}
static int rebin_plan(kid_handle *h, bool dead_last) {
  const bool carry_repro = h->rp.srows_n == h->n;
  rows_moved(h, dead_last);
  const long long n = h->n;
  const unsigned nb = (unsigned)((n + 255) / 256);
  const unsigned dead_key = (unsigned)h->ncell;
  { const int rc_s = perm_storage(h); if (rc_s) return rc_s; }
  const int32_t *live = nullptr;
  { const int rc_l = layout_flags(h, &live); if (rc_l) return rc_l; }
  const unsigned *perm = nullptr;
  if (h->stable_resort) {
    unsigned bits = 1; while ((1ull << bits) <= (unsigned long long)dead_key) ++bits;
    hipLaunchKernelGGL(cell_key_kernel, dim3(nb), dim3(256), 0, h->stream, h->bp.i[KID_BI_INE], h->bp.i[KID_BI_JNE], live,
                       h->gd.isd, h->gd.jsd, h->ni, dead_key, h->d_key[0], h->d_idx[0], n);
    size_t tmp = h->sort_tmp.bytes;
    KID_HIP(h, rocprim::radix_sort_pairs(h->sort_tmp.p, tmp, h->d_key[0], h->d_key[1], h->d_idx[0], h->d_idx[1], (size_t)n, 0u, bits, h->stream));
    perm = h->d_idx[1];
  } else {
    KID_HIP(h, hipMemsetAsync(h->d_cell_hist, 0, ((size_t)h->ncell + 1) * sizeof(unsigned), h->stream));
    hipLaunchKernelGGL(cell_rank_kernel, dim3(nb), dim3(256), 0, h->stream, h->bp.i[KID_BI_INE], h->bp.i[KID_BI_JNE], live,
                       h->gd.isd, h->gd.jsd, h->ni, dead_key, h->d_key[0], h->d_key[1], h->d_cell_hist, n);
    size_t tmp = h->cscan_tmp.bytes;
    KID_HIP(h, rocprim::exclusive_scan(h->cscan_tmp.p, tmp, h->d_cell_hist, h->d_cell_hist, 0u, (size_t)h->ncell + 1, rocprim::plus<unsigned>(), h->stream));
    hipLaunchKernelGGL(cell_place_kernel, dim3(nb), dim3(256), 0, h->stream, h->d_key[0], h->d_key[1], h->d_cell_hist, h->d_idx[1], h->d_idx[0], n);
    perm = h->d_idx[1];
    if (carry_repro) { hipLaunchKernelGGL(translate_rows_kernel, dim3(nb), dim3(256), 0, h->stream, h->rp.srows, (const unsigned *)h->d_idx[0], n); h->rp.srows_n = n; }
  }
  perm_fields(h, perm, n);
  KID_HIP(h, hipGetLastError());
  return KID_OK;
}
static int rebin_swap(kid_handle *h) {
  const kid_handle::RebinPlan &pl = h->rplan;
  for (int q = 0; q < pl.nmf; ++q) std::swap(h->bp.f[pl.moved_f[q]], h->bp_alt.f[pl.moved_f[q]]);
  std::swap(h->bp.id, h->bp_alt.id);
  for (int f = 0; f < KID_NB_I32; ++f) std::swap(h->bp.i[f], h->bp_alt.i[f]);
  if (h->tables_dirty) return refresh_tables(h);
  { const int rc = join_side(h); if (rc) return rc; }
  hipLaunchKernelGGL(set_berg_table_kernel, dim3(1), dim3(64), 0, h->stream, h->bp, h->d_bp);
  KID_HIP(h, hipGetLastError());
  return KID_OK;
}
static int rebin_apply(kid_handle *h, bool with_lane, int *list, const int *list_count) {
  PermTable t = h->rplan.t;
  const long long n = h->rplan.n;
  const unsigned nb = (unsigned)((n + 255) / 256);
  if (with_lane) {
    if (h->stable_resort) { h->err = "KID_STABLE_RESORT has no inverse permutation for the slow-lane re-binning"; return KID_EUNSUPPORTED; }
    if (!h->d_lane_alt) KID_HIP(h, h->mem.dev(h->d_lane_alt, (size_t)h->capacity, 0));
    t.src[t.n8 + t.n4] = h->d_lane; t.dst[t.n8 + t.n4] = h->d_lane_alt; ++t.n4;
  }
  if (n > 0) hipLaunchKernelGGL(permute_all_kernel, dim3(nb), dim3(256), 0, h->stream, t, h->rplan.perm, n);
  if (with_lane) {
    std::swap(h->d_lane, h->d_lane_alt);
    if (list) hipLaunchKernelGGL(translate_list_kernel, dim3(64), dim3(256), 0, h->stream, list, list_count, h->d_idx[0]);
  }
  KID_HIP(h, hipGetLastError());
  return rebin_swap(h);
}
static int rebin_flush(kid_handle *h) {
  if (!h->rebin_pending) return KID_OK;
  h->rebin_pending = false;
  KID_HIP(h, hipSetDevice(h->device));
  return rebin_apply(h, false, nullptr, nullptr);
}
static bool rebin_table(const kid_handle *h, int K, RebinTab &tab) {
  const kid_handle::RebinPlan &pl = h->rplan;
  tab = RebinTab{};
  tab.dst = h->bp;
  for (int q = 0; q < pl.nmf; ++q) tab.dst.f[pl.moved_f[q]] = h->bp_alt.f[pl.moved_f[q]];
  tab.dst.id = h->bp_alt.id;
  for (int f = 0; f < KID_NB_I32; ++f) tab.dst.i[f] = h->bp_alt.i[f];
  tab.moved = pl.moved;
  const unsigned long long own = KID_RB_DYN | rb_thermo_fields(K);
  for (int q = 0; q < pl.nmf; ++q) {
    const int f = pl.moved_f[q];
    if ((own >> f) & 1ull) continue;
    if (tab.n8 >= KID_RB_NX8 - 1) { tab.surplus |= 1ull << f; continue; }
    tab.xs[tab.n8] = h->bp.f[f]; tab.xd[tab.n8] = h->bp_alt.f[f]; ++tab.n8;
  }
  tab.xs[tab.n8] = h->bp.id; tab.xd[tab.n8] = h->bp_alt.id; ++tab.n8;
  static_assert(KID_NB_I32 - 2 <= KID_RB_NX4, "every int32 field but the cell is a head copy");
  for (int f = 0; f < KID_NB_I32; ++f) {
    if (f == KID_BI_INE || f == KID_BI_JNE) continue;
    tab.xs[KID_RB_NX8 + tab.n4] = h->bp.i[f]; tab.xd[KID_RB_NX8 + tab.n4] = h->bp_alt.i[f]; ++tab.n4;
  }
  return true;
}
int kid_set_resort_interval(kid_handle *h, int steps) {
  if (!h || steps < 0) return KID_EINVAL;
  h->resort_interval = steps;
  return KID_OK;
}
int kid_perm_moved_fields(kid_handle *h, int64_t *count) {
  if (!h || !count) return KID_EINVAL;
  *count = h->rplan.nmf;
  return KID_OK;
}

}
```

### icebergs_amd/csrc/kid_rows_plan.hpp

```cpp
#pragma once
#include "../../include/kid_types.h"

namespace kid {

enum WireKind { WIRE_F64, WIRE_I32, WIRE_INE, WIRE_JNE, WIRE_ID_HI, WIRE_ID_LO };
struct WireWord { WireKind kind; int field; };
constexpr WireWord WIRE_RECORD[] = {
  {WIRE_F64, KID_B_LON}, {WIRE_F64, KID_B_LAT}, {WIRE_F64, KID_B_UVEL}, {WIRE_F64, KID_B_VVEL},
  {WIRE_F64, KID_B_UVEL_PREV}, {WIRE_F64, KID_B_VVEL_PREV}, {WIRE_F64, KID_B_XI}, {WIRE_F64, KID_B_YJ},
  {WIRE_F64, KID_B_START_LON}, {WIRE_F64, KID_B_START_LAT}, {WIRE_I32, KID_BI_START_YEAR}, {WIRE_F64, KID_B_START_DAY},
  {WIRE_F64, KID_B_START_MASS}, {WIRE_F64, KID_B_MASS}, {WIRE_F64, KID_B_THICKNESS}, {WIRE_F64, KID_B_WIDTH},
  {WIRE_F64, KID_B_LENGTH}, {WIRE_F64, KID_B_FL_K}, {WIRE_F64, KID_B_MASS_SCALING}, {WIRE_F64, KID_B_MASS_OF_BITS},
  {WIRE_F64, KID_B_MASS_OF_FL_BITS}, {WIRE_F64, KID_B_MASS_OF_FL_BERGY_BITS}, {WIRE_F64, KID_B_HEAT_DENSITY},
  {WIRE_INE, KID_BI_INE}, {WIRE_JNE, KID_BI_JNE},
  {WIRE_F64, KID_B_AXN}, {WIRE_F64, KID_B_AYN}, {WIRE_F64, KID_B_BXN}, {WIRE_F64, KID_B_BYN},
  {WIRE_F64, KID_B_HALO_BERG}, {WIRE_F64, KID_B_STATIC_BERG}, {WIRE_ID_HI, -1}, {WIRE_ID_LO, -1},
  {WIRE_F64, KID_B_OD},
};
constexpr int MIG_WIDTH = (int)(sizeof(WIRE_RECORD) / sizeof(WIRE_RECORD[0]));
static_assert(MIG_WIDTH == 34, "buffer_width without bonds, mts and dem (FW:21)");

constexpr int wire_word(WireKind kind, int field) {
  for (int w = 0; w < MIG_WIDTH; ++w)
    if (WIRE_RECORD[w].kind == kind && (WIRE_RECORD[w].field == field || kind >= WIRE_INE)) return w;
  return -1;
}
constexpr int WIRE_W_LON = wire_word(WIRE_F64, KID_B_LON), WIRE_W_LAT = wire_word(WIRE_F64, KID_B_LAT);
constexpr int WIRE_W_UVEL = wire_word(WIRE_F64, KID_B_UVEL), WIRE_W_VVEL = wire_word(WIRE_F64, KID_B_VVEL);
constexpr int WIRE_W_INE = wire_word(WIRE_INE, 0), WIRE_W_JNE = wire_word(WIRE_JNE, 0);
constexpr int WIRE_W_HALO_BERG = wire_word(WIRE_F64, KID_B_HALO_BERG), WIRE_W_STATIC_BERG = wire_word(WIRE_F64, KID_B_STATIC_BERG);
constexpr int WIRE_W_ID_HI = wire_word(WIRE_ID_HI, 0), WIRE_W_ID_LO = wire_word(WIRE_ID_LO, 0), WIRE_W_OD = wire_word(WIRE_F64, KID_B_OD);
static_assert(WIRE_W_INE == 23 && WIRE_W_JNE == 24 && WIRE_W_HALO_BERG == 29 && WIRE_W_ID_HI == 31 && WIRE_W_OD == 33, "the layout of FW:3268-3301");

constexpr bool marks_has_static(int f) { return f == KID_B_STATIC_BERG || f == KID_B_HALO_BERG; }
constexpr bool marks_has_fl(int f) { return f == KID_B_MASS_OF_FL_BITS || f == KID_B_MASS_OF_FL_BERGY_BITS || f == KID_B_FL_K; }

struct NeverWrittenIn { bool footloose, mts, calving_on, periodic_reentry, runge_not_verlet, has_fl, env_ever_stored; };
constexpr bool field_never_written(const NeverWrittenIn &s, int f) {
  if (s.footloose || s.mts || s.calving_on) return false;
  switch (f) {
    case KID_B_AXN_FAST: case KID_B_AYN_FAST: case KID_B_BXN_FAST: case KID_B_BYN_FAST: case KID_B_ANG_VEL: case KID_B_ANG_ACCEL: case KID_B_ROT:
    case KID_B_UVEL_OLD: case KID_B_VVEL_OLD: case KID_B_LON_OLD: case KID_B_LAT_OLD:
      return !s.periodic_reentry;
    case KID_B_HALO_BERG: case KID_B_STATIC_BERG: case KID_B_START_LON: case KID_B_START_LAT: case KID_B_START_MASS: case KID_B_HEAT_DENSITY:
      return true;
    case KID_B_UVEL_PREV: case KID_B_VVEL_PREV:
      return s.runge_not_verlet;
    case KID_B_MASS_OF_FL_BITS: case KID_B_MASS_OF_FL_BERGY_BITS: case KID_B_FL_K: case KID_B_START_DAY: case KID_B_MASS_SCALING:
      return !s.has_fl;
    case KID_B_UO: case KID_B_VO: case KID_B_UI: case KID_B_VI: case KID_B_UA: case KID_B_VA: case KID_B_SSH_X: case KID_B_SSH_Y:
    case KID_B_SST: case KID_B_SSS: case KID_B_CN: case KID_B_HI: case KID_B_OD:
      return !s.env_ever_stored;
    default:
      return false;
  }
}

struct ZeroState {
  bool uploaded_nonzero[KID_NB_F64] = {};
  bool launched_nonzero[KID_NB_F64] = {};
  constexpr void uploaded(int f, bool nonzero) { uploaded_nonzero[f] = nonzero; launched_nonzero[f] = false; }
  constexpr void appended_by_kernel() { for (bool &nz : uploaded_nonzero) nz = true; }
  constexpr void appended_word(int f) { uploaded_nonzero[f] = true; }
  constexpr void launched_accel() { launched_nonzero[KID_B_AXN] = true; launched_nonzero[KID_B_AYN] = true; }
  constexpr void launched_berg(bool evolve, bool thermo, bool rk, bool erosion_zero, bool has_fl, bool footloose) {
    if ((evolve && !rk) || footloose) launched_accel();
    if ((thermo && (!erosion_zero || has_fl)) || footloose) launched_nonzero[KID_B_MASS_OF_BITS] = true;
  }
  constexpr void launched_other() { launched_accel(); launched_nonzero[KID_B_MASS_OF_BITS] = true; }
};
struct KnownZeroIn { bool uploaded_nonzero, launched_nonzero, never_written, rk, erosion_zero; };
constexpr bool field_known_zero(const KnownZeroIn &s, int f) {
  if (s.uploaded_nonzero) return false;
  switch (f) {
    case KID_B_AXN: case KID_B_AYN: return !s.launched_nonzero && s.rk;
    case KID_B_MASS_OF_BITS: return !s.launched_nonzero && s.erosion_zero;
    case KID_B_HEAT_DENSITY: return s.never_written;
    default: return false;
  }
}
constexpr unsigned long long KID_ZERO_FIELDS = (1ull << KID_B_AXN) | (1ull << KID_B_AYN) | (1ull << KID_B_MASS_OF_BITS) | (1ull << KID_B_HEAT_DENSITY);
static_assert(KID_B_AXN < 64 && KID_B_AYN < 64 && KID_B_MASS_OF_BITS < 64 && KID_B_HEAT_DENSITY < 64, "one bit per fp64 field");
constexpr unsigned long long known_zero_mask(const ZeroState &z, bool heat_density_never_written, bool rk, bool erosion_zero) {
  unsigned long long m = 0ull;
  for (int f = 0; f < KID_NB_F64; ++f)
    if (((KID_ZERO_FIELDS >> f) & 1ull) &&
        field_known_zero(KnownZeroIn{z.uploaded_nonzero[f], z.launched_nonzero[f], f == KID_B_HEAT_DENSITY && heat_density_never_written, rk, erosion_zero}, f))
      m |= 1ull << f;
  constexpr unsigned long long accel = (1ull << KID_B_AXN) | (1ull << KID_B_AYN);
  if ((m & accel) != accel) m &= ~accel;
  return m;
}

}
```

### icebergs_amd/framework.py

```python
import atexit
import ctypes as C
import weakref

import numpy as np

from . import lib as _lib
from . import types as T


def _dp(a):
    return a.ctypes.data_as(C.POINTER(C.c_double))


def _chk_record(rec):
    return {name: getattr(rec, name) for name, _ in T.GrdChksum._fields_ if name != "pad_"}


def _a18(txt):
    return txt[:18].rjust(18)


def _es16_9(x):
    if x != x:
        return "NaN".rjust(16)
    if x in (float("inf"), float("-inf")):
        return ("Infinity" if x > 0 else "-Infinity").rjust(16)
    mant, exp = ("%.9E" % x).split("E")
    return (mant + ("E" + exp if len(exp) == 3 else exp)).rjust(16)


def format_bergs_chksum(label, six):
    names = ("chksum", "chksum2", "chksum3", "chksum4", "chksum5", "#")
    return "KID, bergs_chksum: " + _a18(label) + "".join(" %s=%22d" % (n, v) for n, v in zip(names, six))


def format_grd_chksum(label, rec, three_d=False):
    head = "KID, grd_chksum%d: " % (3 if three_d else 2)
    ints = "".join(" %s=%22d" % (n, rec[n]) for n in ("chksum", "chksum2"))
    reals = "".join(" %s=%s" % (n, _es16_9(rec[k])) for n, k in (("min", "minv"), ("max", "maxv"), ("mean", "mean"), ("rms", "rms"), ("sd", "sd")))
    return head + _a18(label) + ints + reals


_LIVE = weakref.WeakSet()


@atexit.register
def _close_live_handles():
    for ib in list(_LIVE):
        try:
            ib.close()
        except Exception:
            pass


class Icebergs:

    def __init__(self, grid, params, capacity, device=0):
        self.lib = _lib.load()
        self.grid = grid
        self.params = params
        self.device = int(device)
        d = grid["desc"]
        self.ni, self.nj = d.ied - d.isd + 1, d.jed - d.jsd + 1
        self.ncell = self.ni * self.nj
        self.h = C.c_void_p()
        rc = self.lib.kid_create(C.byref(d), C.byref(params), int(capacity), int(device), C.byref(self.h))
        if rc != 0:
            msg = self.lib.kid_last_error(self.h).decode() if self.h else "kid_create failed"
            if self.h:
                self.lib.kid_destroy(self.h)
                self.h = None
            raise _lib.KidError("kid_create: rc=%d %s" % (rc, msg))
        arr = (C.POINTER(C.c_double) * T.ENUMS["KID_NGRID_STATIC"])()
        keep = []
        for k, name in enumerate(T.GRID_STATIC_NAMES):
            a = np.ascontiguousarray(grid["static"][name], dtype=np.float64)
            assert a.shape == (self.nj, self.ni), (name, a.shape)
            keep.append(a)
            arr[k] = _dp(a)
        self._check(self.lib.kid_set_static_grid(self.h, arr), "kid_set_static_grid")
        self.set_forcing(grid["forcing"])
        self.acc = np.zeros((T.NACC, self.nj, self.ni))
        self.out = np.zeros((T.NOUT, self.nj, self.ni))
        self.scalars = np.zeros(T.NSCALAR)
        _LIVE.add(self)

    def _check(self, rc, what):
        if rc != 0:
            raise _lib.KidError("%s: rc=%d %s" % (what, rc, self.lib.kid_last_error(self.h).decode()))

    def close(self):
        if getattr(self, "h", None):
            self.lib.kid_destroy(self.h)
            self.h = None
        _LIVE.discard(self)

    def __del__(self):
        try:
            self.close()
        except Exception:
            pass

    def set_forcing(self, forcing):
        arr = (C.POINTER(C.c_double) * T.ENUMS["KID_NFORCING"])()
        keep = []
        for k, name in enumerate(T.FORCING_NAMES):
            a = np.ascontiguousarray(forcing[name], dtype=np.float64)
            assert a.shape == (self.nj, self.ni), (name, a.shape)
            keep.append(a)
            arr[k] = _dp(a)
        self._check(self.lib.kid_set_forcing(self.h, arr), "kid_set_forcing")

    def ingest_forcing(self, args, vel_stagger="B", stress_stagger="B", tau_is_velocity=False, cyclic_x=False, on_device=False):
        if on_device:
            key = (tuple(sorted((k, int(v[0]), tuple(v[1])) for k, v in args.items() if v is not None)), vel_stagger, stress_stagger, bool(tau_is_velocity), bool(cyclic_x))
            if getattr(self, "_ingest_key", None) == key:
                self._check(self.lib.kid_ingest_forcing(self.h, self._ingest_ref), "kid_ingest_forcing")
                return
        st = {"B": T.ENUMS["KID_BGRID_NE"], "C": T.ENUMS["KID_CGRID_NE"], "A": T.ENUMS["KID_AGRID"]}
        fin, keep, shape = T.ForcingIn(), [], {}
        for name in ("uo", "vo", "ui", "vi", "tauxa", "tauya", "ssh", "sst", "cn", "hi", "sss"):
            v = args.get(name)
            if v is None:
                setattr(fin, name, None)
                continue
            if on_device:
                ptr, shp = v
                setattr(fin, name, C.cast(C.c_void_p(int(ptr)), C.POINTER(C.c_double)))
            else:
                a = np.ascontiguousarray(v, dtype=np.float64)
                keep.append(a)
                shp = a.shape
                setattr(fin, name, _dp(a))
            shape[name] = shp
        for name, other in (("uo", "ui"), ("vo", "vi")):
            assert shape[name] == shape[other], (name, other)
        d = self.grid["desc"]
        nic, njc = d.iec - d.isc + 1, d.jec - d.jsc + 1
        for name in ("ssh", "cn", "hi"):
            assert shape[name] == (njc + 2, nic + 2), (name, shape[name])
        for name in ("sst", "sss"):
            assert name not in shape or shape[name] == (njc, nic), (name, shape[name])
        fin.u_nj, fin.u_ni = shape["uo"]
        fin.v_nj, fin.v_ni = shape["vo"]
        fin.taux_nj, fin.taux_ni = shape["tauxa"]
        fin.tauy_nj, fin.tauy_ni = shape["tauya"]
        fin.vel_stagger, fin.stress_stagger = st[vel_stagger], st[stress_stagger]
        fin.tau_is_velocity, fin.cyclic_x, fin.on_device = int(tau_is_velocity), int(cyclic_x), int(on_device)
        self._check(self.lib.kid_ingest_forcing(self.h, C.byref(fin)), "kid_ingest_forcing")
        if on_device:
            self._ingest_key, self._ingest_fin, self._ingest_ref = key, fin, C.byref(fin)

    def get_forcing(self):
        out = {name: np.empty((self.nj, self.ni)) for name in T.FORCING_NAMES}
        arr = (C.POINTER(C.c_double) * T.ENUMS["KID_NFORCING"])(*[_dp(out[name]) for name in T.FORCING_NAMES])
        self._check(self.lib.kid_get_forcing(self.h, arr), "kid_get_forcing")
        return out

    def set_traj_params(self, tp):
        self._check(self.lib.kid_set_traj_params(self.h, C.byref(tp)), "kid_set_traj_params")

    def record_posn(self):
        self._check(self.lib.kid_record_posn(self.h), "kid_record_posn")

    def num_traj_records(self):
        n = C.c_int64()
        self._check(self.lib.kid_num_traj_records(self.h, C.byref(n)), "kid_num_traj_records")
        return n.value

    def write_trajectories(self, path):
        self._check(self.lib.kid_write_trajectories(self.h, str(path).encode()), "kid_write_trajectories")

    def num_bond_traj_records(self):
        n = C.c_int64()
        self._check(self.lib.kid_num_bond_traj_records(self.h, C.byref(n)), "kid_num_bond_traj_records")
        return n.value

    def write_bond_trajectories(self, path):
        self._check(self.lib.kid_write_bond_trajectories(self.h, str(path).encode()), "kid_write_bond_trajectories")

    def buffer_width(self):
        w = C.c_int32()
        self._check(self.lib.kid_buffer_width(self.h, C.byref(w)), "kid_buffer_width")
        return w.value

    def pack_emigrants(self, direction):
        n = C.c_int64()
        if getattr(self, "_mig_buf", None) is None:
            self._mig_buf = np.empty((4096, self.buffer_width()))
        rc = self.lib.kid_pack_emigrants(self.h, direction, _dp(self._mig_buf), self._mig_buf.shape[0], C.byref(n))
        if rc == -4 and n.value > self._mig_buf.shape[0]:
            self._mig_buf = np.empty((2 * n.value, self._mig_buf.shape[1]))
            rc = self.lib.kid_pack_emigrants(self.h, direction, _dp(self._mig_buf), self._mig_buf.shape[0], C.byref(n))
        self._check(rc, "kid_pack_emigrants")
        return self._mig_buf[:n.value].copy()

    def pack_emigrants_pair(self, axis):
        na, nb = C.c_int64(), C.c_int64()
        if getattr(self, "_mig_buf2", None) is None:
            self._mig_buf2 = [np.empty((4096, self.buffer_width())) for _ in range(2)]
        for attempt in range(2):
            a, b = self._mig_buf2
            rc = self.lib.kid_pack_emigrants_pair(self.h, axis, _dp(a), a.shape[0], C.byref(na), _dp(b), b.shape[0], C.byref(nb))
            if rc != -4 or attempt:
                break
            self._mig_buf2 = [np.empty((max(2 * n.value, x.shape[0]), x.shape[1])) for n, x in ((na, a), (nb, b))]
        self._check(rc, "kid_pack_emigrants_pair")
        return self._mig_buf2[0][:na.value].copy(), self._mig_buf2[1][:nb.value].copy()

    def unpack_immigrants_pair(self, buf_a, buf_b):
        a, b = (np.ascontiguousarray(x, dtype=np.float64) for x in (buf_a, buf_b))
        if a.size or b.size:
            self._check(self.lib.kid_unpack_immigrants_pair(self.h, _dp(a) if a.size else None, a.shape[0] if a.size else 0,
                                                            _dp(b) if b.size else None, b.shape[0] if b.size else 0), "kid_unpack_immigrants_pair")

    def pack_halo_bergs_pair(self, axis, width=0, sides=(True, True)):
        n = [C.c_int64(), C.c_int64()]
        if getattr(self, "_halo_berg_buf", None) is None:
            self._halo_berg_buf = [np.empty((4096, 34)) for _ in range(2)]
        for attempt in range(2):
            a, b = self._halo_berg_buf
            rc = self.lib.kid_pack_halo_bergs_pair(self.h, int(axis), int(width), _dp(a) if sides[0] else None, a.shape[0], C.byref(n[0]),
                                                   _dp(b) if sides[1] else None, b.shape[0], C.byref(n[1]))
            if rc != -4 or attempt:
                break
            self._halo_berg_buf = [np.empty((max(2 * q.value, x.shape[0]), 34)) for q, x in zip(n, (a, b))]
        self._check(rc, "kid_pack_halo_bergs_pair")
        return self._halo_berg_buf[0][:n[0].value].copy(), self._halo_berg_buf[1][:n[1].value].copy()

    def halo_berg_count(self):
        n = C.c_int64()
        self._check(self.lib.kid_halo_berg_count(self.h, C.byref(n)), "kid_halo_berg_count")
        return n.value

    def unpack_immigrants(self, buf):
        buf = np.ascontiguousarray(buf, dtype=np.float64)
        if buf.size:
            self._check(self.lib.kid_unpack_immigrants(self.h, _dp(buf), buf.shape[0]), "kid_unpack_immigrants")

    def calculate_mass_on_ocean(self):
        self._check(self.lib.kid_calculate_mass_on_ocean(self.h), "kid_calculate_mass_on_ocean")

    def halo_plane_count(self):
        n = C.c_int32()
        self._check(self.lib.kid_halo_plane_count(self.h, C.byref(n)), "kid_halo_plane_count")
        return n.value

    def halo_buffer_count(self, axis, width=1):
        n = C.c_int64()
        self._check(self.lib.kid_halo_buffer_count(self.h, int(axis), int(width), C.byref(n)), "kid_halo_buffer_count")
        return n.value

    def _halo_buffers(self, bufs, count, what):
        ptrs, dev = [], None
        for b in bufs:
            if b is None:
                ptrs.append(None)
                continue
            on_dev = not isinstance(b, np.ndarray)
            assert dev is None or dev == on_dev, what + ": both buffers on the host or both on the device"
            dev = on_dev
            if on_dev:
                import torch
                assert isinstance(b, torch.Tensor) and b.is_cuda and b.device.index == self.device and b.dtype == torch.float64 and b.is_contiguous(), what
                assert b.numel() == count, (what, b.numel(), count)
                ptrs.append(b.data_ptr())
            else:
                assert b.dtype == np.float64 and b.flags.c_contiguous and b.size == count, (what, b.shape, count)
                ptrs.append(b.ctypes.data)
        return ptrs, bool(dev)

    def _halo_order_in(self, bufs):
        import torch
        torch.cuda.current_stream(next(b for b in bufs if b is not None).device).synchronize()

    def pack_halo_pair(self, axis, width=1, out=None):
        count = self.halo_buffer_count(axis, width)
        if out is None:
            out = (np.empty(count), np.empty(count))
        ptrs, dev = self._halo_buffers(out, count, "pack_halo_pair")
        if dev:
            self._halo_order_in(out)
        self._check(self.lib.kid_pack_halo_pair(self.h, int(axis), int(width), ptrs[0], ptrs[1], int(dev)), "kid_pack_halo_pair")
        if dev:
            self.sync()
        return tuple(out)

    def unpack_halo_pair(self, axis, from_lo, from_hi, width=1):
        count = self.halo_buffer_count(axis, width)
        bufs = (from_lo, from_hi)
        if from_lo is None and from_hi is None:
            return
        ptrs, dev = self._halo_buffers(bufs, count, "unpack_halo_pair")
        if dev:
            self._halo_order_in(bufs)
        self._check(self.lib.kid_unpack_halo_pair(self.h, int(axis), int(width), ptrs[0], ptrs[1], int(dev)), "kid_unpack_halo_pair")
        if dev:
            self.sync()

    def unpack_halo_fold(self, from_fold, width=1, swap_slots=True):
        count = self.halo_buffer_count(1, width)
        assert from_fold is not None, "unpack_halo_fold: a fold tile always has a partner"
        ptrs, dev = self._halo_buffers((from_fold,), count, "unpack_halo_fold")
        if dev:
            self._halo_order_in((from_fold,))
        self._check(self.lib.kid_unpack_halo_fold(self.h, int(width), ptrs[0], int(bool(swap_slots)), int(dev)), "kid_unpack_halo_fold")
        if dev:
            self.sync()

    def fold_halo_self(self, width=1, swap_slots=True):
        self._check(self.lib.kid_fold_halo_self(self.h, int(width), int(bool(swap_slots))), "kid_fold_halo_self")

    def write_restart(self, directory):
        self._check(self.lib.kid_write_restart(self.h, str(directory).encode()), "kid_write_restart")

    def read_restart(self, directory):
        self._check(self.lib.kid_read_restart(self.h, str(directory).encode()), "kid_read_restart")

    LOCATE_MODES = {"search": 1, "scan": 2}

    def locate_bergs(self, mode="search"):
        if mode not in self.LOCATE_MODES:
            raise ValueError("locate_bergs: mode is 'search' or 'scan', not %r" % (mode,))
        c = (C.c_int64 * 3)()
        self._check(self.lib.kid_locate_bergs(self.h, self.LOCATE_MODES[mode], c), "kid_locate_bergs")
        return {"found": int(c[0]), "lost": int(c[1]), "grounded": int(c[2])}

    def set_restart_locate(self, mode):
        if mode is not None and mode not in self.LOCATE_MODES:
            raise ValueError("set_restart_locate: mode is None, 'search' or 'scan', not %r" % (mode,))
        self._check(self.lib.kid_set_restart_locate(self.h, 0 if mode is None else self.LOCATE_MODES[mode]), "kid_set_restart_locate")

    def set_calving_params(self, cp):
        self._calv_params = cp
        self._check(self.lib.kid_set_calving_params(self.h, C.byref(cp)), "kid_set_calving_params")

    def set_calving_state(self, stored_ice=None, stored_heat=None, rmean_calving=None, rmean_calving_hflx=None):
        arrs = [None if a is None else np.ascontiguousarray(a, dtype=np.float64) for a in (stored_ice, stored_heat, rmean_calving, rmean_calving_hflx)]
        if arrs[0] is not None:
            assert arrs[0].shape == (T.ENUMS["KID_NCLASSES"], self.nj, self.ni)
        self._check(self.lib.kid_set_calving_state(self.h, *[None if a is None else _dp(a) for a in arrs]), "kid_set_calving_state")

    def get_calving_state(self):
        nk = T.ENUMS["KID_NCLASSES"]
        out = {"stored_ice": np.empty((nk, self.nj, self.ni)), "stored_heat": np.empty((self.nj, self.ni)),
               "rmean_calving": np.empty((self.nj, self.ni)), "rmean_calving_hflx": np.empty((self.nj, self.ni)),
               "real_calving": np.empty((nk, self.nj, self.ni)), "calving": np.empty((self.nj, self.ni)), "calving_hflx": np.empty((self.nj, self.ni))}
        self._check(self.lib.kid_get_calving_state(self.h, _dp(out["stored_ice"]), _dp(out["stored_heat"]), _dp(out["rmean_calving"]),
                                                   _dp(out["rmean_calving_hflx"]), _dp(out["real_calving"])), "kid_get_calving_state")
        self._check(self.lib.kid_get_calving(self.h, _dp(out["calving"]), _dp(out["calving_hflx"])), "kid_get_calving")
        return out

    def calving(self, calving, calving_hflx, on_device=False):
        cin = T.CalvingIn()
        if on_device:
            cin.calving = C.cast(C.c_void_p(int(calving)), C.POINTER(C.c_double))
            cin.calving_hflx = C.cast(C.c_void_p(int(calving_hflx)), C.POINTER(C.c_double))
        else:
            d = self.grid["desc"]
            a = np.ascontiguousarray(calving, dtype=np.float64)
            b = np.ascontiguousarray(calving_hflx, dtype=np.float64)
            assert a.shape == b.shape == (d.jec - d.jsc + 1, d.iec - d.isc + 1), a.shape
            cin.calving, cin.calving_hflx = _dp(a), _dp(b)
        cin.on_device = int(on_device)
        scal = np.zeros(T.ENUMS["KID_NCALV_SCALARS"])
        self._check(self.lib.kid_calving(self.h, C.byref(cin), _dp(scal)), "kid_calving")
        return scal

    def set_forcing_device(self, dev_ptrs):
        arr = (C.c_void_p * T.ENUMS["KID_NFORCING"])(*[C.c_void_p(int(x)) if x else None for x in dev_ptrs])
        self._check(self.lib.kid_set_forcing_device(self.h, arr), "kid_set_forcing_device")

    def step_prepare(self, dev_ptrs=None):
        if dev_ptrs is None:
            self._check(self.lib.kid_step_prepare(self.h, None), "kid_step_prepare")
            return
        key = tuple(int(x) if x else 0 for x in dev_ptrs)
        if getattr(self, "_prep_key", None) != key:
            self._prep_key = key
            self._prep_arr = (C.c_void_p * T.ENUMS["KID_NFORCING"])(*[C.c_void_p(x) if x else None for x in key])
        self._check(self.lib.kid_step_prepare(self.h, self._prep_arr), "kid_step_prepare")

    def set_params(self, params):
        self.params = params
        self._check(self.lib.kid_set_params(self.h, C.byref(params)), "kid_set_params")

    def set_side_stream(self, stream_ptr, enable=True):
        self._check(self.lib.kid_set_side_stream(self.h, C.c_void_p(stream_ptr), int(enable)), "kid_set_side_stream")

    def set_stream(self, stream_ptr):
        self._check(self.lib.kid_set_stream(self.h, C.c_void_p(stream_ptr)), "kid_set_stream")

    @staticmethod
    def _soa(bergs, n=None):
        s = T.BergSoA()
        s.n = len(bergs["lon"]) if n is None else n
        for k, name in enumerate(T.BERG_F64_NAMES):
            a = bergs[name]
            assert a.dtype == np.float64 and a.flags.c_contiguous
            s.f64[k] = _dp(a)
        for k, name in enumerate(T.BERG_I32_NAMES):
            a = bergs[name]
            assert a.dtype == np.int32 and a.flags.c_contiguous
            s.i32[k] = a.ctypes.data_as(C.POINTER(C.c_int32))
        s.id = bergs["id"].ctypes.data_as(C.POINTER(C.c_int64))
        return s

    def upload_bergs(self, bergs):
        s = self._soa(bergs, bergs.get("_n"))
        self._check(self.lib.kid_upload_bergs(self.h, C.byref(s)), "kid_upload_bergs")

    @staticmethod
    def _bond_soa(bonds, n):
        s = T.BondSoA()
        s.n, s.max_bonds = n, int(bonds["max_bonds"])
        assert len(bonds["count"]) == n and bonds["count"].dtype == np.int32
        s.count = bonds["count"].ctypes.data_as(C.POINTER(C.c_int32))
        s.other_id = bonds["other_id"].ctypes.data_as(C.POINTER(C.c_int64))
        s.broken = bonds["broken"].ctypes.data_as(C.POINTER(C.c_int32))
        for k, name in enumerate(T.BOND_F64_NAMES):
            a = bonds[name]
            assert a.dtype == np.float64 and len(a) == s.max_bonds * n
            s.f64[k] = _dp(a)
        return s

    def upload_bonds(self, bonds):
        n, _ = self.num_bergs()
        self._check(self.lib.kid_upload_bonds(self.h, C.byref(self._bond_soa(bonds, n))), "kid_upload_bonds")

    def download_bonds(self, max_bonds):
        from .synthetic import empty_bonds
        n, _ = self.num_bergs()
        bd = empty_bonds(n, max_bonds)
        self._check(self.lib.kid_download_bonds(self.h, C.byref(self._bond_soa(bd, n))), "kid_download_bonds")
        return bd

    def initialize_bonds(self, from_radii=True, length=None):
        if not from_radii and length is None:
            raise ValueError("initialize_bonds: give a length or use from_radii")
        n = C.c_int64()
        self._check(self.lib.kid_initialize_bonds(self.h, 1 if from_radii else 0, 0.0 if length is None else float(length), C.byref(n)),
                    "kid_initialize_bonds")
        return n.value

    def count_bonds(self):
        a, b = C.c_int64(), C.c_int64()
        self._check(self.lib.kid_count_bonds(self.h, C.byref(a), C.byref(b)), "kid_count_bonds")
        return a.value, b.value

    def set_conglom_ids(self):
        self._check(self.lib.kid_set_conglom_ids(self.h), "kid_set_conglom_ids")

    def evolve_icebergs_mts(self):
        self._check(self.lib.kid_evolve_icebergs_mts(self.h), "kid_evolve_icebergs_mts")

    def num_bergs(self):
        a, b = C.c_int64(), C.c_int64()
        self._check(self.lib.kid_num_bergs(self.h, C.byref(a), C.byref(b)), "kid_num_bergs")
        return a.value, b.value

    def download_bergs(self):
        from .synthetic import empty_bergs
        n, _ = self.num_bergs()
        b = empty_bergs(n)
        s = self._soa(b)
        self._check(self.lib.kid_download_bergs(self.h, C.byref(s)), "kid_download_bergs")
        return b

    def set_store_environment(self, on):
        self._check(self.lib.kid_set_store_environment(self.h, 1 if on else 0), "kid_set_store_environment")

    def set_reproducible_sums(self, on):
        self._check(self.lib.kid_set_reproducible_sums(self.h, 1 if on else 0), "kid_set_reproducible_sums")

    def bergs_chksum(self):
        out = (C.c_int64 * 6)()
        self._check(self.lib.kid_bergs_chksum(self.h, out), "kid_bergs_chksum")
        return tuple(int(v) for v in out)

    def bergs_chksum_device(self, per_cell=False):
        out, rec = (C.c_int64 * 6)(), T.GrdChksum()
        self._check(self.lib.kid_bergs_chksum_device(self.h, out, C.byref(rec) if per_cell else None), "kid_bergs_chksum_device")
        six = tuple(int(v) for v in out)
        return (six, _chk_record(rec)) if per_cell else six

    def checksum_gridded(self):
        recs = (T.GrdChksum * T.NCHK)()
        self._check(self.lib.kid_checksum_gridded(self.h, recs, T.NCHK), "kid_checksum_gridded")
        return {label: _chk_record(recs[k]) for k, label in enumerate(T.CHK_LABELS)}

    def checksum_report(self, label):
        six, per_cell = self.bergs_chksum_device(per_cell=True)
        lines = [format_bergs_chksum(label, six), format_grd_chksum("# of bergs/cell", per_cell), "KID: checksumming gridded data @ " + label.rstrip()]
        for name, rec in self.checksum_gridded().items():
            if rec["present"]:
                lines.append(format_grd_chksum(name, rec, three_d=name in T.CHK_3D))
        return lines

    def stock(self, index):
        v = C.c_double()
        self._check(self.lib.kid_stock(self.h, int(index), C.byref(v)), "kid_stock")
        return v.value

    def budget(self):
        out = T.BudgetOut()
        self._check(self.lib.kid_budget(self.h, C.byref(out)), "kid_budget")
        return {name: getattr(out, name) for name, _ in T.BudgetOut._fields_}

    def incr_mass(self, plane):
        if isinstance(plane, np.ndarray):
            assert plane.dtype == np.float64 and plane.flags.c_contiguous and plane.ndim == 2, "float64, C-contiguous, 2-d"
            self._check(self.lib.kid_incr_mass(self.h, plane.ctypes.data, 0, plane.shape[1], plane.shape[0]), "kid_incr_mass")
            return plane
        import torch
        assert isinstance(plane, torch.Tensor) and plane.is_cuda and plane.dtype == torch.float64 and plane.is_contiguous() and plane.dim() == 2
        assert plane.device.index == self.device, "the tensor lives on another device than the handle"
        torch.cuda.current_stream(plane.device).synchronize()
        self._check(self.lib.kid_incr_mass(self.h, plane.data_ptr(), 1, plane.shape[1], plane.shape[0]), "kid_incr_mass")
        self.sync()
        return plane

    def set_footloose_step(self, step):
        self._check(self.lib.kid_set_footloose_step(self.h, int(step)), "kid_set_footloose_step")

    def get_footloose_step(self):
        s = C.c_int64(0)
        self._check(self.lib.kid_get_footloose_step(self.h, C.byref(s)), "kid_get_footloose_step")
        return int(s.value)

    def adjust_fl_berg_interactivity(self):
        n = C.c_int64(0)
        self._check(self.lib.kid_adjust_fl_berg_interactivity(self.h, C.byref(n)), "kid_adjust_fl_berg_interactivity")
        return int(n.value)

    def set_iceberg_counter(self, counter):
        a = np.ascontiguousarray(counter, dtype=np.int32)
        assert a.shape == (self.nj, self.ni)
        self._check(self.lib.kid_set_iceberg_counter(self.h, a.ctypes.data_as(C.POINTER(C.c_int32))), "kid_set_iceberg_counter")

    def get_iceberg_counter(self):
        a = np.zeros((self.nj, self.ni), dtype=np.int32)
        self._check(self.lib.kid_get_iceberg_counter(self.h, a.ctypes.data_as(C.POINTER(C.c_int32))), "kid_get_iceberg_counter")
        return a

    def move_berg_between_cells(self):
        self._check(self.lib.kid_move_berg_between_cells(self.h), "kid_move_berg_between_cells")

    def set_resort_interval(self, steps):
        self._check(self.lib.kid_set_resort_interval(self.h, int(steps)), "kid_set_resort_interval")

    def compact(self):
        self._check(self.lib.kid_compact_bergs(self.h), "kid_compact_bergs")

    @property
    def capacity(self):
        n = C.c_int64()
        self._check(self.lib.kid_capacity(self.h, C.byref(n)), "kid_capacity")
        return n.value

    def reserve(self, rows):
        self._check(self.lib.kid_reserve(self.h, int(rows)), "kid_reserve")

    def set_auto_reserve(self, min_free, growth=1.5, max_capacity=0):
        self._check(self.lib.kid_set_auto_reserve(self.h, int(min_free), float(growth), int(max_capacity)), "kid_set_auto_reserve")

    def run(self, nsteps=1):
        self._check(self.lib.kid_run_step(self.h, int(nsteps)), "kid_run_step")

    def step_local(self):
        self._check(self.lib.kid_step_local(self.h), "kid_step_local")

    def step_gather(self):
        self._check(self.lib.kid_step_gather(self.h), "kid_step_gather")

    def run_phases(self, nsteps=1):
        p = self.params
        for _ in range(nsteps):
            self._check(self.lib.kid_zero_accumulators(self.h), "kid_zero_accumulators")
            if not p.mts and not p.old_interp_flds_order:
                self._check(self.lib.kid_interp_gridded_fields_to_bergs(self.h), "interp")
            self._check(self.lib.kid_evolve_icebergs(self.h), "kid_evolve_icebergs")
            if p.footloose:
                self._check(self.lib.kid_footloose_calving(self.h), "kid_footloose_calving")
            if not p.old_interp_flds_order:
                self._check(self.lib.kid_interp_gridded_fields_to_bergs(self.h), "interp")
            self._check(self.lib.kid_thermodynamics(self.h), "kid_thermodynamics")
            self._check(self.lib.kid_create_gridded_icebergs_fields(self.h), "kid_create_gridded")

    def fetch(self):
        self._check(self.lib.kid_get_accumulators(self.h, _dp(self.acc), _dp(self.out), _dp(self.scalars)), "kid_get_accumulators")
        return self.acc, self.out, self.scalars

    def sync(self):
        self._check(self.lib.kid_sync(self.h), "kid_sync")

    def accum_device_ptr(self):
        p, n = C.c_void_p(), C.c_int64()
        self._check(self.lib.kid_accum_device_ptr(self.h, C.byref(p), C.byref(n)), "kid_accum_device_ptr")
        return p.value, n.value

    def accum_live_count(self):
        n = C.c_int64()
        self._check(self.lib.kid_accum_live_count(self.h, C.byref(n)), "kid_accum_live_count")
        return n.value

    def bind_accum_buffer(self, ptr, count):
        self._check(self.lib.kid_bind_accum_buffer(self.h, C.c_void_p(ptr), int(count)), "kid_bind_accum_buffer")

    def bind_spread_mass_old(self, ptr, count):
        self._check(self.lib.kid_bind_spread_mass_old(self.h, ptr, int(count)), "kid_bind_spread_mass_old")

    def last_redo_count(self):
        c = C.c_int64()
        self._check(self.lib.kid_last_redo_count(self.h, C.byref(c)), "kid_last_redo_count")
        return c.value

    def rebin_fused_count(self):
        c = C.c_int64()
        self._check(self.lib.kid_rebin_fused_count(self.h, C.byref(c)), "kid_rebin_fused_count")
        return c.value

    def hot_zero_mask(self):
        m = C.c_uint64()
        self._check(self.lib.kid_hot_zero_mask(self.h, C.byref(m)), "kid_hot_zero_mask")
        return {name for f, name in enumerate(T.BERG_F64_NAMES) if (m.value >> f) & 1}

    def profile(self, on=True):
        self._check(self.lib.kid_profile_enable(self.h, 1 if on else 0), "kid_profile_enable")

    def profile_get(self):
        a, n, b = C.c_double(), C.c_int64(), C.c_double()
        self._check(self.lib.kid_profile_get(self.h, C.byref(a), C.byref(n), C.byref(b)), "kid_profile_get")
        return a.value, n.value, b.value
```

### icebergs_amd/lib.py

```python
import ctypes as C
import os
import subprocess

from . import types as T

_CSRC = os.path.join(os.path.dirname(os.path.abspath(__file__)), "csrc")
SO_PATH = os.environ.get("KID_HIP_SO", os.path.join(_CSRC, "libkid_hip.so"))

SYMBOLS = [
    "kid_create", "kid_destroy", "kid_memory_in_use", "kid_set_params", "kid_set_stream", "kid_sync", "kid_last_error", "kid_version",
    "kid_sizeof", "kid_set_static_grid", "kid_set_forcing", "kid_set_forcing_device", "kid_upload_bergs", "kid_download_bergs",
    "kid_num_bergs", "kid_compact_bergs", "kid_move_berg_between_cells", "kid_set_resort_interval", "kid_capacity", "kid_reserve", "kid_set_auto_reserve", "kid_zero_accumulators", "kid_interp_gridded_fields_to_bergs",
    "kid_evolve_icebergs", "kid_footloose_calving", "kid_set_footloose_step", "kid_get_footloose_step", "kid_footloose_uniform", "kid_adjust_fl_berg_interactivity", "kid_thermodynamics", "kid_create_gridded_icebergs_fields",
    "kid_set_store_environment", "kid_set_reproducible_sums", "kid_set_iceberg_counter", "kid_get_iceberg_counter", "kid_step_local", "kid_step_gather", "kid_run_step", "kid_get_accumulators", "kid_accum_device_ptr", "kid_accum_live_count",
    "kid_bind_accum_buffer", "kid_bind_spread_mass_old", "kid_profile_enable", "kid_profile_get",
    "kid_last_redo_count", "kid_rebin_fused_count", "kid_hot_zero_mask", "kid_set_side_stream", "kid_step_prepare", "kid_upload_bonds", "kid_download_bonds", "kid_evolve_icebergs_mts", "kid_set_conglom_ids", "kid_evolve_icebergs_interactive",
    "kid_initialize_bonds", "kid_count_bonds",
    "kid_budget", "kid_stock", "kid_incr_mass",
    "kid_ingest_forcing", "kid_get_forcing",
    "kid_set_calving_params", "kid_set_calving_state", "kid_get_calving_state", "kid_calving", "kid_get_calving",
    "kid_restart_write_bergs", "kid_restart_count_bergs", "kid_restart_read_bergs", "kid_restart_write_bonds", "kid_restart_read_bonds", "kid_write_restart", "kid_read_restart", "kid_bergs_chksum",
    "kid_bergs_chksum_device", "kid_checksum_gridded",
    "kid_locate_bergs", "kid_set_restart_locate",
    "kid_set_traj_params", "kid_record_posn", "kid_num_traj_records", "kid_write_trajectories",
    "kid_num_bond_traj_records", "kid_write_bond_trajectories",
    "kid_buffer_width", "kid_pack_emigrants", "kid_unpack_immigrants", "kid_pack_emigrants_pair", "kid_unpack_immigrants_pair",
    "kid_pack_halo_bergs_pair", "kid_halo_berg_count",
    "kid_calculate_mass_on_ocean", "kid_halo_plane_count", "kid_halo_buffer_count", "kid_pack_halo_pair", "kid_unpack_halo_pair",
    "kid_unpack_halo_fold", "kid_fold_halo_self",
]


class KidError(RuntimeError):
    pass


def build(verbose=False):
    subprocess.run(["make", "-C", _CSRC, "-j2", "all"] + ([] if verbose else ["-s"]), check=True)
    return SO_PATH


def device_reset():
    C.CDLL("libamdhip64.so").hipDeviceReset()


_lib = None


def load():
    global _lib
    if _lib is not None:
        return _lib
    if not os.path.exists(SO_PATH):
        raise KidError("libkid_hip.so is not built (run `python -c 'import __graft_entry__ as g; g.build()'`); "
                       "there is no CPU fallback")
    import torch
    lib = C.CDLL(SO_PATH)
    H = C.c_void_p
    dp = C.POINTER(C.c_double)
    lib.kid_version.restype = C.c_char_p
    lib.kid_last_error.restype = C.c_char_p
    lib.kid_last_error.argtypes = [H]
    lib.kid_sizeof.restype = C.c_int64
    lib.kid_sizeof.argtypes = [C.c_int]
    lib.kid_create.argtypes = [C.POINTER(T.GridDesc), C.POINTER(T.Params), C.c_int64, C.c_int, C.POINTER(H)]
    lib.kid_destroy.argtypes = [H]
    lib.kid_memory_in_use.argtypes = [C.POINTER(C.c_int64), C.POINTER(C.c_int64)]
    lib.kid_set_params.argtypes = [H, C.POINTER(T.Params)]
    lib.kid_set_stream.argtypes = [H, C.c_void_p]
    lib.kid_sync.argtypes = [H]
    lib.kid_set_static_grid.argtypes = [H, C.POINTER(dp)]
    lib.kid_set_forcing.argtypes = [H, C.POINTER(dp)]
    lib.kid_set_forcing_device.argtypes = [H, C.POINTER(C.c_void_p)]
    lib.kid_ingest_forcing.argtypes = [H, C.POINTER(T.ForcingIn)]
    lib.kid_get_forcing.argtypes = [H, C.POINTER(dp)]
    lib.kid_set_calving_params.argtypes = [H, C.POINTER(T.CalvingParams)]
    lib.kid_set_calving_state.argtypes = [H, dp, dp, dp, dp]
    lib.kid_get_calving_state.argtypes = [H, dp, dp, dp, dp, dp]
    lib.kid_calving.argtypes = [H, C.POINTER(T.CalvingIn), dp]
    lib.kid_get_calving.argtypes = [H, dp, dp]
    lib.kid_restart_write_bergs.argtypes = [C.c_char_p, C.POINTER(T.Params), C.POINTER(T.BergSoA)]
    lib.kid_restart_count_bergs.argtypes = [C.c_char_p, C.POINTER(C.c_int64)]
    lib.kid_restart_read_bergs.argtypes = [C.c_char_p, C.POINTER(T.BergSoA), C.c_int64]
    lib.kid_restart_write_bonds.argtypes = [C.c_char_p, C.POINTER(T.Params), C.POINTER(T.BergSoA), C.POINTER(T.BondSoA)]
    lib.kid_restart_read_bonds.argtypes = [C.c_char_p, C.POINTER(T.BergSoA), C.POINTER(T.BondSoA)]
    lib.kid_write_restart.argtypes = [H, C.c_char_p]
    lib.kid_set_traj_params.argtypes = [H, C.POINTER(T.TrajParams)]
    lib.kid_record_posn.argtypes = [H]
    lib.kid_num_traj_records.argtypes = [H, C.POINTER(C.c_int64)]
    lib.kid_write_trajectories.argtypes = [H, C.c_char_p]
    lib.kid_num_bond_traj_records.argtypes = [H, C.POINTER(C.c_int64)]
    lib.kid_write_bond_trajectories.argtypes = [H, C.c_char_p]
    lib.kid_buffer_width.argtypes = [H, C.POINTER(C.c_int32)]
    lib.kid_pack_emigrants.argtypes = [H, C.c_int32, C.POINTER(C.c_double), C.c_int64, C.POINTER(C.c_int64)]
    lib.kid_unpack_immigrants.argtypes = [H, C.POINTER(C.c_double), C.c_int64]
    lib.kid_pack_emigrants_pair.argtypes = [H, C.c_int32, C.POINTER(C.c_double), C.c_int64, C.POINTER(C.c_int64), C.POINTER(C.c_double), C.c_int64, C.POINTER(C.c_int64)]
    lib.kid_unpack_immigrants_pair.argtypes = [H, C.POINTER(C.c_double), C.c_int64, C.POINTER(C.c_double), C.c_int64]
    lib.kid_pack_halo_bergs_pair.argtypes = [H, C.c_int32, C.c_int32, C.POINTER(C.c_double), C.c_int64, C.POINTER(C.c_int64), C.POINTER(C.c_double), C.c_int64, C.POINTER(C.c_int64)]
    lib.kid_halo_berg_count.argtypes = [H, C.POINTER(C.c_int64)]
    lib.kid_calculate_mass_on_ocean.argtypes = [H]
    lib.kid_halo_plane_count.argtypes = [H, C.POINTER(C.c_int32)]
    lib.kid_halo_buffer_count.argtypes = [H, C.c_int32, C.c_int32, C.POINTER(C.c_int64)]
    lib.kid_pack_halo_pair.argtypes = [H, C.c_int32, C.c_int32, C.c_void_p, C.c_void_p, C.c_int32]
    lib.kid_unpack_halo_pair.argtypes = [H, C.c_int32, C.c_int32, C.c_void_p, C.c_void_p, C.c_int32]
    lib.kid_unpack_halo_fold.argtypes = [H, C.c_int32, C.c_void_p, C.c_int32, C.c_int32]
    lib.kid_fold_halo_self.argtypes = [H, C.c_int32, C.c_int32]
    lib.kid_read_restart.argtypes = [H, C.c_char_p]
    older = ("kid_rebin_fused_count", "kid_hot_zero_mask", "kid_locate_bergs", "kid_set_restart_locate", "kid_bergs_chksum_device", "kid_checksum_gridded")
    if hasattr(lib, "kid_locate_bergs"):
        lib.kid_locate_bergs.argtypes = [H, C.c_int, C.POINTER(C.c_int64)]
        lib.kid_set_restart_locate.argtypes = [H, C.c_int]
    lib.kid_upload_bergs.argtypes = [H, C.POINTER(T.BergSoA)]
    lib.kid_step_prepare.argtypes = [H, C.POINTER(C.c_void_p)]
    lib.kid_set_side_stream.argtypes = [H, C.c_void_p, C.c_int]
    lib.kid_last_redo_count.argtypes = [H, C.POINTER(C.c_int64)]
    if hasattr(lib, "kid_rebin_fused_count"):
        lib.kid_rebin_fused_count.argtypes = [H, C.POINTER(C.c_int64)]
    if hasattr(lib, "kid_hot_zero_mask"):
        lib.kid_hot_zero_mask.argtypes = [H, C.POINTER(C.c_uint64)]
    lib.kid_upload_bonds.argtypes = [H, C.POINTER(T.BondSoA)]
    lib.kid_download_bonds.argtypes = [H, C.POINTER(T.BondSoA)]
    lib.kid_evolve_icebergs_mts.argtypes = [H]
    lib.kid_set_conglom_ids.argtypes = [H]
    lib.kid_initialize_bonds.argtypes = [H, C.c_int32, C.c_double, C.POINTER(C.c_int64)]
    lib.kid_count_bonds.argtypes = [H, C.POINTER(C.c_int64), C.POINTER(C.c_int64)]
    lib.kid_budget.argtypes = [H, C.POINTER(T.BudgetOut)]
    lib.kid_stock.argtypes = [H, C.c_int32, C.POINTER(C.c_double)]
    lib.kid_incr_mass.argtypes = [H, C.c_void_p, C.c_int32, C.c_int32, C.c_int32]
    lib.kid_evolve_icebergs_interactive.argtypes = [H]
    lib.kid_download_bergs.argtypes = [H, C.POINTER(T.BergSoA)]
    lib.kid_num_bergs.argtypes = [H, C.POINTER(C.c_int64), C.POINTER(C.c_int64)]
    lib.kid_set_resort_interval.argtypes = [H, C.c_int]
    lib.kid_capacity.argtypes = [H, C.POINTER(C.c_int64)]
    lib.kid_reserve.argtypes = [H, C.c_int64]
    lib.kid_set_auto_reserve.argtypes = [H, C.c_int64, C.c_double, C.c_int64]
    for name in ("kid_compact_bergs", "kid_move_berg_between_cells", "kid_zero_accumulators", "kid_interp_gridded_fields_to_bergs",
                 "kid_evolve_icebergs", "kid_footloose_calving", "kid_thermodynamics",
                 "kid_create_gridded_icebergs_fields", "kid_step_local", "kid_step_gather"):
        getattr(lib, name).argtypes = [H]
    lib.kid_run_step.argtypes = [H, C.c_int]
    lib.kid_set_store_environment.argtypes = [H, C.c_int]
    lib.kid_set_reproducible_sums.argtypes = [H, C.c_int]
    lib.kid_bergs_chksum.argtypes = [H, C.POINTER(C.c_int64)]
    if hasattr(lib, "kid_bergs_chksum_device"):
        lib.kid_bergs_chksum_device.argtypes = [H, C.POINTER(C.c_int64), C.POINTER(T.GrdChksum)]
        lib.kid_checksum_gridded.argtypes = [H, C.POINTER(T.GrdChksum), C.c_int32]
    lib.kid_footloose_uniform.argtypes = [C.c_int32, C.c_int64, C.c_int64, C.c_int32]
    lib.kid_set_footloose_step.argtypes = [H, C.c_int64]
    lib.kid_get_footloose_step.argtypes = [H, C.POINTER(C.c_int64)]
    lib.kid_adjust_fl_berg_interactivity.argtypes = [H, C.POINTER(C.c_int64)]
    lib.kid_set_iceberg_counter.argtypes = [H, C.POINTER(C.c_int32)]
    lib.kid_get_iceberg_counter.argtypes = [H, C.POINTER(C.c_int32)]
    lib.kid_get_accumulators.argtypes = [H, dp, dp, dp]
    lib.kid_accum_device_ptr.argtypes = [H, C.POINTER(C.c_void_p), C.POINTER(C.c_int64)]
    lib.kid_accum_live_count.argtypes = [H, C.POINTER(C.c_int64)]
    lib.kid_bind_accum_buffer.argtypes = [H, C.c_void_p, C.c_int64]
    lib.kid_bind_spread_mass_old.argtypes = [H, C.c_void_p, C.c_int64]
    lib.kid_profile_enable.argtypes = [H, C.c_int]
    lib.kid_profile_get.argtypes = [H, dp, C.POINTER(C.c_int64), dp]
    for name in SYMBOLS:
        if name in older and not hasattr(lib, name):
            continue
        if name not in ("kid_version", "kid_last_error", "kid_sizeof", "kid_footloose_uniform"):
            getattr(lib, name).restype = C.c_int
    lib.kid_footloose_uniform.restype = C.c_double
    assert lib.kid_sizeof(0) == C.sizeof(T.Params), "kid_params layout mismatch between header and library"
    assert lib.kid_sizeof(1) == C.sizeof(T.GridDesc)
    assert lib.kid_sizeof(2) == C.sizeof(T.BergSoA)
    assert lib.kid_sizeof(3) == C.sizeof(T.BondSoA)
    assert lib.kid_sizeof(4) == C.sizeof(T.ForcingIn)
    assert lib.kid_sizeof(5) == C.sizeof(T.CalvingParams) and lib.kid_sizeof(6) == C.sizeof(T.CalvingIn)
    _lib = lib
    return lib
```

Measured before the change: 11.79 billion berg-steps/s.

## Defer permuting cold berg fields during re-binning via an origin index

When bergs are re-sorted by cell, fields the step kernel never reads (start position, id, fast-rotation terms, conglomerate id and so on, depending on the namelist) are no longer permuted every sort. An origin index is carried through the permutations and the cold fields are gathered once, on demand, when a reader or a config change needs them. This cuts the bytes moved per re-sort and frees slots in the fused rebin table. The per-cell rank kernel is also rewritten from a sorted-run head scan to a match-any style loop that groups equal keys anywhere in the wavefront. The cost is more bookkeeping, an extra int32 array per row, and some risk of stale fields if a reader skips materialisation.

```diff
diff --git a/icebergs_amd/csrc/kid_handle.hpp b/icebergs_amd/csrc/kid_handle.hpp
--- a/icebergs_amd/csrc/kid_handle.hpp
+++ b/icebergs_amd/csrc/kid_handle.hpp
@@ -79,7 +79,7 @@
   int side_mode = 0; int *d_lane = nullptr, *d_lane_alt = nullptr; hipEvent_t evR = nullptr; int lane_step = 1; bool lanes_active = false, carry_valid = false, evC_live = false;
   hipEvent_t evC = nullptr, evP = nullptr;
   ForcingSet fset[2]; int forc_parity = 0;
-  struct DebugOpts { bool stable_resort = false, no_plain_build = false, fl_unfused = false, new_order_unfused = false, mts_always_label = false, mts_no_fused = false, rebin_eager = false, chksum_timing = false, no_zero_skip = false;
+  struct DebugOpts { bool stable_resort = false, no_plain_build = false, fl_unfused = false, new_order_unfused = false, mts_always_label = false, mts_no_fused = false, rebin_eager = false, chksum_timing = false, no_zero_skip = false, cold_eager = false;
                      int mts_fused_blocks_cap = 0, mts_poll_limit = 0; } dbg;
   int32_t *d_iceberg_counter = nullptr;
   bool fl_place_warm = false;
@@ -92,7 +92,9 @@
   BergPtrs bp_alt{};
   bool rebin_pending = false;
   int64_t rebin_fused_count = 0;
-  struct RebinPlan { PermTable t{}; int moved_f[KID_NB_F64] = {}; int nmf = 0; unsigned long long moved = 0ull, zero_skipped = 0ull; const unsigned *perm = nullptr; long long n = 0; } rplan;
+  struct RebinPlan { PermTable t{}; int moved_f[KID_NB_F64] = {}; int nmf = 0; unsigned long long moved = 0ull, zero_skipped = 0ull; const unsigned *perm = nullptr; long long n = 0;
+                     unsigned moved_i32 = 0u; bool moved_id = false, origin_moves = false; } rplan;
+  struct ColdState { kid::ColdSet set; bool deferred = false; int64_t materialised = 0; int32_t *origin = nullptr, *origin_alt = nullptr; } cold;
   RebinTab *d_rb = nullptr;
   unsigned *d_cell_hist = nullptr; Scratch cscan_tmp; bool stable_resort = false;
   int resort_interval = 16, steps_since_sort = 0;
@@ -149,6 +151,8 @@
 extern "C" {
 static int refresh_tables(kid_handle *h), join_side(kid_handle *h);
 static int rebin_flush(kid_handle *h);
+static int rebin_flush_rows(kid_handle *h);
+static int cold_materialise(kid_handle *h), cold_settle(kid_handle *h);
 static int rebin_plan(kid_handle *h, bool dead_last);
 static int rebin_core(kid_handle *h, bool with_lane, int *list, const int *list_count), rebin_apply(kid_handle *h, bool with_lane, int *list, const int *list_count);
 static bool plain_namelist(const kid_handle *h), lanes_eligible(const kid_handle *h);
diff --git a/icebergs_amd/csrc/kid_hip.hip b/icebergs_amd/csrc/kid_hip.hip
--- a/icebergs_amd/csrc/kid_hip.hip
+++ b/icebergs_amd/csrc/kid_hip.hip
@@ -152,7 +152,7 @@
   h->dbg.stable_resort = getenv("KID_STABLE_RESORT") != nullptr; h->dbg.no_plain_build = getenv("KID_NO_PLAIN_BUILD") != nullptr;
   h->dbg.fl_unfused = getenv("KID_FL_UNFUSED") != nullptr; h->dbg.new_order_unfused = getenv("KID_NEW_ORDER_UNFUSED") != nullptr;
   h->dbg.rebin_eager = getenv("KID_REBIN_EAGER") != nullptr; h->dbg.chksum_timing = getenv("KID_CHKSUM_TIMING") != nullptr;
-  h->dbg.no_zero_skip = getenv("KID_NO_ZERO_SKIP") != nullptr;
+  h->dbg.no_zero_skip = getenv("KID_NO_ZERO_SKIP") != nullptr; h->dbg.cold_eager = getenv("KID_COLD_EAGER") != nullptr;
   h->dbg.mts_always_label = getenv("KID_MTS_ALWAYS_LABEL") != nullptr; h->dbg.mts_no_fused = getenv("KID_MTS_NO_FUSED") != nullptr;
   if (const char *e = getenv("KID_MTS_FUSED_BLOCKS_CAP")) h->dbg.mts_fused_blocks_cap = atoi(e);
   if (const char *e = getenv("KID_MTS_POLL_LIMIT")) h->dbg.mts_poll_limit = atoi(e);
@@ -233,7 +233,7 @@
   h->labels_stale = true;
   h->flags.footprint = footprint_needed(h->params) ? 1 : 0;
   if (!h->params.old_interp_flds_order && !h->env_off_requested) h->flags.store_env = 1;
-  return KID_OK;
+  return cold_settle(h);
 }
 static int join_side(kid_handle *h) {
   for (int q = 0; q < 2; ++q)
@@ -335,7 +335,7 @@
   if (!h) return KID_EINVAL;
   h->flags.store_env = on ? 1 : 0;
   h->env_off_requested = !on;
-  return KID_OK;
+  return cold_settle(h);
 }
 
 static int refresh_tables(kid_handle *h) {
diff --git a/icebergs_amd/csrc/kid_launch.inc b/icebergs_amd/csrc/kid_launch.inc
--- a/icebergs_amd/csrc/kid_launch.inc
+++ b/icebergs_amd/csrc/kid_launch.inc
@@ -96,9 +96,14 @@
 static int rebin_take_or_flush(kid_handle *h, bool whole, RebinTab &rtab, bool &fused) {
   fused = false;
   if (!h->rebin_pending) return KID_OK;
-  fused = PH == PH_STEP && rebin_fusable(h) && whole && h->rplan.n == h->n && (h->rplan.zero_skipped & ~known_zero_mask(h)) == 0ull &&
+  fused = PH == PH_STEP && rebin_fusable(h) && whole && h->rplan.n == h->n && (h->rplan.zero_skipped & ~known_zero_mask(h)) == 0ull && cold_holds(h) &&
           rebin_table(h, h->flags.store_env ? 3 : 1, rtab);
-  return fused ? KID_OK : rebin_flush(h);
+  return fused ? KID_OK : rebin_flush_rows(h);
+}
+template <unsigned PH>
+static int cold_for_launch(kid_handle *h) {
+  if (!h->cold.deferred || (PH == PH_STEP && rebin_fusable(h) && cold_holds(h))) return KID_OK;
+  return cold_materialise(h);
 }
 static int rebin_bind(kid_handle *h, const RebinTab &rtab, Redo &redo) {
   hipLaunchKernelGGL(set_rebin_table_kernel, dim3(1), dim3(64), 0, h->stream, rtab, h->d_rb);
@@ -160,6 +165,7 @@
   RebinTab rtab;
   bool rebin_fused = false;
   if (!rc) rc = rebin_take_or_flush<PH>(h, whole, rtab, rebin_fused);
+  if (!rc) rc = cold_for_launch<PH>(h);
   if (!rc) rc = refresh_tables(h);
   if (rc) return rc;
   const BergLaunch c = berg_launch(h);
@@ -375,6 +381,7 @@
   h->acc_prezeroed = false;
   if (!rc) rc = repro_refuse(h);
   if (!rc && h->rebin_pending && !rebin_fusable(h)) rc = rebin_flush(h);
+  if (!rc && !rebin_fusable(h)) rc = cold_materialise(h);
   if (rc) return rc;
   const kid_params &p = h->params;
   if (p.mts) return step_mts(h);
diff --git a/icebergs_amd/csrc/kid_reserve.inc b/icebergs_amd/csrc/kid_reserve.inc
--- a/icebergs_amd/csrc/kid_reserve.inc
+++ b/icebergs_amd/csrc/kid_reserve.inc
@@ -94,6 +94,7 @@
   for (auto &field : h->bp_alt.f) L.add(field, RESERVE_LAZY);
   for (auto &field : h->bp_alt.i) L.add(field, RESERVE_LAZY);
   L.add(h->bp_alt.id, RESERVE_LAZY);
+  for (int32_t **q : {&h->cold.origin, &h->cold.origin_alt}) L.add(*q, RESERVE_LAZY);
   for (unsigned **q : {&h->d_key[0], &h->d_key[1], &h->d_idx[0], &h->d_idx[1], &h->d_cell_hist}) L.add(*q, RESERVE_LAZY);
   for (Scratch *t : {&h->sort_tmp, &h->scan_tmp, &h->cscan_tmp}) L.add(*t, RESERVE_LAZY);
   L.add(h->d_lane_alt, RESERVE_LAZY);
diff --git a/icebergs_amd/csrc/kid_rows.inc b/icebergs_amd/csrc/kid_rows.inc
--- a/icebergs_amd/csrc/kid_rows.inc
+++ b/icebergs_amd/csrc/kid_rows.inc
@@ -48,17 +48,25 @@
   const bool in = k < n;
   const unsigned c = in ? (alive[k] ? (unsigned)((ine[k] - isd) + (jne[k] - jsd) * ni) : dead_key) : 0xffffffffu;
   const int lane = (int)__lane_id();
-  const unsigned prev = __shfl_up(c, 1);
-  const bool head = (lane == 0) || (prev != c);
-  const unsigned long long heads = __ballot(head);
-  const unsigned long long below = heads & ((lane == 63) ? ~0ull : ((2ull << lane) - 1ull));
-  const int head_lane = 63 - __clzll(below);
-  const unsigned long long above = (lane == 63) ? 0ull : (heads >> (lane + 1));
-  const int next_head = above ? lane + 1 + (__ffsll((long long)above) - 1) : 64;
+  unsigned long long rem = __ballot(in);
+  int leader = lane;
+  unsigned cnt = 0u, place = 0u;
+  while (rem != 0ull) {
+    const int u = (int)__ffsll((long long)rem) - 1;
+    const unsigned cu = (unsigned)__builtin_amdgcn_readlane((int)c, u);
+    const bool mine = in && c == cu;
+    const unsigned long long bm = __ballot(mine);
+    if (mine) { leader = u; cnt = (unsigned)__popcll(bm); place = __builtin_amdgcn_mbcnt_hi((unsigned)(bm >> 32), __builtin_amdgcn_mbcnt_lo((unsigned)bm, 0u)); }
+    rem &= ~bm;
+  }
   unsigned base = 0u;
-  if (head && in) base = atomicAdd(hist + c, (unsigned)(next_head - lane));
-  base = __shfl(base, head_lane);
-  if (in) { key[k] = c; rank[k] = base + (unsigned)(lane - head_lane); }
+  if (in && lane == leader) base = atomicAdd(hist + c, cnt);
+  base = __shfl(base, leader);
+  if (in) { key[k] = c; rank[k] = base + place; }
+}
+__global__ void __launch_bounds__(256) iota_i32_kernel(int32_t *p, long long n) {
+  const long long k = (long long)blockIdx.x * 256ll + threadIdx.x;
+  if (k < n) p[k] = (int32_t)k;
 }
 __global__ void __launch_bounds__(256) cell_place_kernel(const unsigned *key, const unsigned *rank, const unsigned *start, unsigned *perm, unsigned *inv, long long n) {
   const long long k = (long long)blockIdx.x * 256ll + threadIdx.x;
@@ -151,10 +159,12 @@
 }
 
 enum RowsMode { ROWS_READ, ROWS_CHANGE };
-static int rows_enter(kid_handle *h, RowsMode mode) {
+enum RowsCold { COLD_READ, COLD_LEAVE };
+static int rows_enter(kid_handle *h, RowsMode mode, RowsCold cold = COLD_READ) {
   KID_HIP(h, hipSetDevice(h->device));
   const int rc = mode == ROWS_CHANGE ? lanes_drain(h) : join_side(h);
-  return rc ? rc : rebin_flush(h);
+  if (rc) return rc;
+  return cold == COLD_LEAVE ? rebin_flush_rows(h) : rebin_flush(h);
 }
 static int count_rows(kid_handle *h, const int32_t *flags, const double *halo, int64_t *count) {
   unsigned long long cnt = 0;
@@ -184,7 +194,7 @@
 
 int kid_num_bergs(kid_handle *h, int64_t *n_slots, int64_t *n_alive) {
   if (!h) return KID_EINVAL;
-  { const int rc = rows_enter(h, ROWS_READ); if (rc) return rc; }
+  { const int rc = rows_enter(h, ROWS_READ, COLD_LEAVE); if (rc) return rc; }
   if (n_slots) *n_slots = h->n;
   if (n_alive) {
     int64_t cnt = 0;
@@ -196,6 +206,7 @@
       { const int rc = count_rows(h, flags, nullptr, &cnt); if (rc) return rc; }
     }
     if (h->tail_valid && cnt < h->n) {
+      { const int rc = cold_materialise(h); if (rc) return rc; }
       rows_truncated(h, cnt);
       if (n_slots) *n_slots = h->n;
     }
@@ -211,6 +222,43 @@
 static unsigned long long known_zero_mask(const kid_handle *h) {
   if (h->dbg.no_zero_skip) return 0ull;
   return kid::known_zero_mask(h->zs, field_never_written(h, KID_B_HEAT_DENSITY), h->params.Runge_not_Verlet != 0, h->params.bergy_bit_erosion_fraction == 0.);
+}
+static bool rebin_fusable(const kid_handle *h);
+static kid::ColdSet cold_set(const kid_handle *h) {
+  const kid_params &p = h->params;
+  if (h->dbg.cold_eager) return kid::ColdSet{};
+  return kid::cold_set(kid::ColdIn{rebin_fusable(h), p.Runge_not_Verlet != 0, p.periodic_reentry != 0, h->flags.has_static != 0, h->flags.has_fl != 0,
+                                   p.iceberg_bonds_on != 0, (p.diag_mask & KID_DIAG_MELT_BY_CLASS) != 0});
+}
+static int berg_table_follows(kid_handle *h) {
+  if (h->tables_dirty) return refresh_tables(h);
+  { const int rc = join_side(h); if (rc) return rc; }
+  hipLaunchKernelGGL(set_berg_table_kernel, dim3(1), dim3(64), 0, h->stream, h->bp, h->d_bp);
+  KID_HIP(h, hipGetLastError());
+  return KID_OK;
+}
+static int cold_materialise(kid_handle *h) {
+  if (!h->cold.deferred) return KID_OK;
+  KID_HIP(h, hipSetDevice(h->device));
+  { const int rc = rebin_flush_rows(h); if (rc) return rc; }
+  h->cold.deferred = false;
+  const kid::ColdSet cs = h->cold.set;
+  h->cold.set = kid::ColdSet{};
+  h->cold.materialised++;
+  PermTable t{};
+  for (int f = 0; f < KID_NB_F64; ++f) if ((cs.f64 >> f) & 1ull) { t.src[t.n8] = h->bp.f[f]; t.dst[t.n8] = h->bp_alt.f[f]; ++t.n8; std::swap(h->bp.f[f], h->bp_alt.f[f]); }
+  if (cs.id) { t.src[t.n8] = h->bp.id; t.dst[t.n8] = h->bp_alt.id; ++t.n8; std::swap(h->bp.id, h->bp_alt.id); }
+  for (int f = 0; f < KID_NB_I32; ++f) if ((cs.i32 >> f) & 1u) { t.src[t.n8 + t.n4] = h->bp.i[f]; t.dst[t.n8 + t.n4] = h->bp_alt.i[f]; ++t.n4; std::swap(h->bp.i[f], h->bp_alt.i[f]); }
+  const long long n = h->n;
+  if (n > 0) hipLaunchKernelGGL(permute_all_kernel, dim3((unsigned)((n + 255) / 256)), dim3(256), 0, h->stream, t, (const unsigned *)h->cold.origin, n);
+  KID_HIP(h, hipGetLastError());
+  return berg_table_follows(h);
+}
+static bool cold_holds(const kid_handle *h) { return !h->cold.deferred || h->cold.set.within(cold_set(h)); }
+static int cold_settle(kid_handle *h) {
+  if (cold_holds(h)) return KID_OK;
+  const int rc = rebin_flush_rows(h);
+  return rc ? rc : cold_materialise(h);
 }
 static int perm_storage(kid_handle *h) {
   if (h->d_key[0]) return KID_OK;
@@ -229,21 +277,37 @@
   for (auto &field : h->bp_alt.f) KID_HIP(h, h->mem.dev(field, (size_t)h->capacity));
   for (auto &field : h->bp_alt.i) KID_HIP(h, h->mem.dev(field, (size_t)h->capacity));
   KID_HIP(h, h->mem.dev(h->bp_alt.id, (size_t)h->capacity));
-  return KID_OK;
-}
-static void perm_fields(kid_handle *h, const unsigned *perm, long long n) {
+  for (int32_t **q : {&h->cold.origin, &h->cold.origin_alt}) KID_HIP(h, h->mem.dev(*q, (size_t)h->capacity));
+  return KID_OK;
+}
+static int perm_fields(kid_handle *h, const unsigned *perm, long long n, bool defer_cold) {
   kid_handle::RebinPlan &pl = h->rplan;
   pl = kid_handle::RebinPlan{};
   PermTable &t = pl.t;
+  kid::ColdSet cold = h->cold.deferred ? h->cold.set : (defer_cold ? cold_set(h) : kid::ColdSet{});
+  if (!h->cold.deferred) {
+    for (int f = 0; f < KID_NB_F64; ++f) if (!h->zs.uploaded_nonzero[f] && field_never_written(h, f)) cold.f64 &= ~(1ull << f);
+  }
+  if (!h->cold.deferred && !cold.empty()) {
+    hipLaunchKernelGGL(iota_i32_kernel, dim3((unsigned)((h->n + 255) / 256)), dim3(256), 0, h->stream, h->cold.origin, (long long)h->n);
+    KID_HIP(h, hipGetLastError());
+    h->cold.deferred = true; h->cold.set = cold;
+  }
   const unsigned long long zeros = known_zero_mask(h);
   for (int f = 0; f < KID_NB_F64; ++f) {
     if (!h->zs.uploaded_nonzero[f] && field_never_written(h, f)) continue;
     if ((zeros >> f) & 1ull) { pl.zero_skipped |= 1ull << f; continue; }
+    if ((cold.f64 >> f) & 1ull) continue;
     t.src[t.n8] = h->bp.f[f]; t.dst[t.n8] = h->bp_alt.f[f]; ++t.n8; pl.moved_f[pl.nmf++] = f; pl.moved |= 1ull << f;
   }
-  t.src[t.n8] = h->bp.id; t.dst[t.n8] = h->bp_alt.id; ++t.n8;
-  for (int f = 0; f < KID_NB_I32; ++f) { t.src[t.n8 + t.n4] = h->bp.i[f]; t.dst[t.n8 + t.n4] = h->bp_alt.i[f]; ++t.n4; }
+  if (!cold.id) { t.src[t.n8] = h->bp.id; t.dst[t.n8] = h->bp_alt.id; ++t.n8; pl.moved_id = true; }
+  for (int f = 0; f < KID_NB_I32; ++f) {
+    if ((cold.i32 >> f) & 1u) continue;
+    t.src[t.n8 + t.n4] = h->bp.i[f]; t.dst[t.n8 + t.n4] = h->bp_alt.i[f]; ++t.n4; pl.moved_i32 |= 1u << f;
+  }
+  if (h->cold.deferred) { t.src[t.n8 + t.n4] = h->cold.origin; t.dst[t.n8 + t.n4] = h->cold.origin_alt; ++t.n4; pl.origin_moves = true; }
   pl.perm = perm; pl.n = n;
+  return KID_OK;
 }
 static const char *const bonds_keep_rows = "bergs with bonds keep their rows: no re-binning while bond tables exist";
 
@@ -266,7 +330,7 @@
   int64_t kept = 0;
   { const int rc = count_rows(h, live, nullptr, &kept); if (rc) return rc; }
   rows_moved(h, false);
-  perm_fields(h, perm, kept);
+  { const int rc = perm_fields(h, perm, kept, false); if (rc) return rc; }
   { const int rc = rebin_apply(h, false, nullptr, nullptr); if (rc) return rc; }
   rows_truncated(h, kept);
   return KID_OK;
@@ -280,7 +344,8 @@
 int kid_move_berg_between_cells(kid_handle *h) {
   if (!h) return KID_EINVAL;
   { const int rc_h = halo_rows_refuse(h, "kid_move_berg_between_cells"); if (rc_h) return rc_h; }
-  { const int rc_e = rows_enter(h, ROWS_CHANGE); if (rc_e) return rc_e; }
+  { const int rc_e = rows_enter(h, ROWS_CHANGE, COLD_LEAVE); if (rc_e) return rc_e; }
+  { const int rc_c = cold_settle(h); if (rc_c) return rc_c; }
   h->steps_since_sort = 0;
   if (h->n == 0) return KID_OK;
   if (h->have_bonds) { h->err = bonds_keep_rows; return KID_EUNSUPPORTED; }
@@ -321,20 +386,16 @@
     perm = h->d_idx[1];
     if (carry_repro) { hipLaunchKernelGGL(translate_rows_kernel, dim3(nb), dim3(256), 0, h->stream, h->rp.srows, (const unsigned *)h->d_idx[0], n); h->rp.srows_n = n; }
   }
-  perm_fields(h, perm, n);
-  KID_HIP(h, hipGetLastError());
-  return KID_OK;
+  KID_HIP(h, hipGetLastError());
+  return perm_fields(h, perm, n, true);
 }
 static int rebin_swap(kid_handle *h) {
   const kid_handle::RebinPlan &pl = h->rplan;
   for (int q = 0; q < pl.nmf; ++q) std::swap(h->bp.f[pl.moved_f[q]], h->bp_alt.f[pl.moved_f[q]]);
-  std::swap(h->bp.id, h->bp_alt.id);
-  for (int f = 0; f < KID_NB_I32; ++f) std::swap(h->bp.i[f], h->bp_alt.i[f]);
-  if (h->tables_dirty) return refresh_tables(h);
-  { const int rc = join_side(h); if (rc) return rc; }
-  hipLaunchKernelGGL(set_berg_table_kernel, dim3(1), dim3(64), 0, h->stream, h->bp, h->d_bp);
-  KID_HIP(h, hipGetLastError());
-  return KID_OK;
+  if (pl.moved_id) std::swap(h->bp.id, h->bp_alt.id);
+  for (int f = 0; f < KID_NB_I32; ++f) if ((pl.moved_i32 >> f) & 1u) std::swap(h->bp.i[f], h->bp_alt.i[f]);
+  if (pl.origin_moves) std::swap(h->cold.origin, h->cold.origin_alt);
+  return berg_table_follows(h);
 }
 static int rebin_apply(kid_handle *h, bool with_lane, int *list, const int *list_count) {
   PermTable t = h->rplan.t;
@@ -353,33 +414,43 @@
   KID_HIP(h, hipGetLastError());
   return rebin_swap(h);
 }
-static int rebin_flush(kid_handle *h) {
+static int rebin_flush_rows(kid_handle *h) {
   if (!h->rebin_pending) return KID_OK;
   h->rebin_pending = false;
   KID_HIP(h, hipSetDevice(h->device));
   return rebin_apply(h, false, nullptr, nullptr);
+}
+static int rebin_flush(kid_handle *h) {
+  const int rc = rebin_flush_rows(h);
+  return rc ? rc : cold_materialise(h);
 }
 static bool rebin_table(const kid_handle *h, int K, RebinTab &tab) {
   const kid_handle::RebinPlan &pl = h->rplan;
   tab = RebinTab{};
   tab.dst = h->bp;
   for (int q = 0; q < pl.nmf; ++q) tab.dst.f[pl.moved_f[q]] = h->bp_alt.f[pl.moved_f[q]];
-  tab.dst.id = h->bp_alt.id;
-  for (int f = 0; f < KID_NB_I32; ++f) tab.dst.i[f] = h->bp_alt.i[f];
+  if (pl.moved_id) tab.dst.id = h->bp_alt.id;
+  for (int f = 0; f < KID_NB_I32; ++f) if ((pl.moved_i32 >> f) & 1u) tab.dst.i[f] = h->bp_alt.i[f];
   tab.moved = pl.moved;
+  const int id_slot = pl.moved_id ? 1 : 0;
   const unsigned long long own = KID_RB_DYN | rb_thermo_fields(K);
   for (int q = 0; q < pl.nmf; ++q) {
     const int f = pl.moved_f[q];
     if ((own >> f) & 1ull) continue;
-    if (tab.n8 >= KID_RB_NX8 - 1) { tab.surplus |= 1ull << f; continue; }
+    if (tab.n8 >= KID_RB_NX8 - id_slot) { tab.surplus |= 1ull << f; continue; }
     tab.xs[tab.n8] = h->bp.f[f]; tab.xd[tab.n8] = h->bp_alt.f[f]; ++tab.n8;
   }
-  tab.xs[tab.n8] = h->bp.id; tab.xd[tab.n8] = h->bp_alt.id; ++tab.n8;
+  if (pl.moved_id) { tab.xs[tab.n8] = h->bp.id; tab.xd[tab.n8] = h->bp_alt.id; ++tab.n8; }
   static_assert(KID_NB_I32 - 2 <= KID_RB_NX4, "every int32 field but the cell is a head copy");
+  static_assert((kid::cold_set(kid::ColdIn{true, true, true, true, true, true, true}).i32 & ~(1u << KID_BI_INE | 1u << KID_BI_JNE)) != 0u, "a cold int32 field makes room for origin");
+  int n4 = 0;
+  for (int f = 0; f < KID_NB_I32; ++f) if (f != KID_BI_INE && f != KID_BI_JNE && ((pl.moved_i32 >> f) & 1u)) ++n4;
+  if (n4 + (pl.origin_moves ? 1 : 0) > KID_RB_NX4) return false;
   for (int f = 0; f < KID_NB_I32; ++f) {
-    if (f == KID_BI_INE || f == KID_BI_JNE) continue;
+    if (f == KID_BI_INE || f == KID_BI_JNE || !((pl.moved_i32 >> f) & 1u)) continue;
     tab.xs[KID_RB_NX8 + tab.n4] = h->bp.i[f]; tab.xd[KID_RB_NX8 + tab.n4] = h->bp_alt.i[f]; ++tab.n4;
   }
+  if (pl.origin_moves) { tab.xs[KID_RB_NX8 + tab.n4] = h->cold.origin; tab.xd[KID_RB_NX8 + tab.n4] = h->cold.origin_alt; ++tab.n4; }
   return true;
 }
 int kid_set_resort_interval(kid_handle *h, int steps) {
@@ -392,5 +463,11 @@
   *count = h->rplan.nmf;
   return KID_OK;
 }
-
-}
+int kid_cold_state(kid_handle *h, int32_t *deferred, int64_t *materialised_count) {
+  if (!h) return KID_EINVAL;
+  if (deferred) *deferred = h->cold.deferred ? 1 : 0;
+  if (materialised_count) *materialised_count = h->cold.materialised;
+  return KID_OK;
+}
+
+}
diff --git a/icebergs_amd/csrc/kid_rows_plan.hpp b/icebergs_amd/csrc/kid_rows_plan.hpp
--- a/icebergs_amd/csrc/kid_rows_plan.hpp
+++ b/icebergs_amd/csrc/kid_rows_plan.hpp
@@ -92,4 +92,57 @@
   return m;
 }
 
+struct ColdIn { bool fusable, runge_not_verlet, periodic_reentry, has_static, has_fl, bonds_on, melt_by_class; };
+constexpr bool step_touches_f64(const ColdIn &s, int f) {
+  switch (f) {
+    case KID_B_START_LON: case KID_B_START_LAT:
+    case KID_B_AXN_FAST: case KID_B_AYN_FAST: case KID_B_BXN_FAST: case KID_B_BYN_FAST: case KID_B_ANG_VEL: case KID_B_ANG_ACCEL: case KID_B_ROT:
+      return false;
+    case KID_B_UVEL_PREV: case KID_B_VVEL_PREV:
+      return !s.runge_not_verlet;
+    case KID_B_UVEL_OLD: case KID_B_VVEL_OLD: case KID_B_LON_OLD: case KID_B_LAT_OLD:
+      return s.periodic_reentry;
+    case KID_B_HALO_BERG: case KID_B_STATIC_BERG:
+      return s.has_static;
+    case KID_B_MASS_OF_FL_BITS: case KID_B_MASS_OF_FL_BERGY_BITS: case KID_B_FL_K:
+    case KID_B_START_DAY:
+      return s.has_fl;
+    case KID_B_START_MASS:
+      return s.melt_by_class;
+    default:
+      return true;
+  }
 }
+constexpr bool step_touches_i32(const ColdIn &s, int f) {
+  switch (f) {
+    case KID_BI_START_YEAR: return s.has_fl;
+    case KID_BI_N_BONDS: return s.bonds_on;
+    case KID_BI_CONGLOM_ID: return false;
+    default: return true;
+  }
+}
+static_assert(KID_NB_I32 <= 32, "one bit per int32 field");
+struct ColdSet {
+  unsigned long long f64 = 0ull; unsigned i32 = 0u; bool id = false;
+  constexpr bool empty() const { return f64 == 0ull && i32 == 0u && !id; }
+  constexpr bool within(const ColdSet &o) const { return (f64 & ~o.f64) == 0ull && (i32 & ~o.i32) == 0u && (!id || o.id); }
+  constexpr int bytes_per_row() const {
+    int b = id ? 8 : 0;
+    for (int f = 0; f < KID_NB_F64; ++f) b += ((f64 >> f) & 1ull) ? 8 : 0;
+    for (int f = 0; f < KID_NB_I32; ++f) b += ((i32 >> f) & 1u) ? 4 : 0;
+    return b;
+  }
+};
+constexpr ColdSet cold_set(const ColdIn &s) {
+  ColdSet c;
+  if (!s.fusable) return c;
+  for (int f = 0; f < KID_NB_F64; ++f) if (!step_touches_f64(s, f)) c.f64 |= 1ull << f;
+  for (int f = 0; f < KID_NB_I32; ++f) if (!step_touches_i32(s, f)) c.i32 |= 1u << f;
+  c.id = true;
+  return c;
+}
+constexpr void origin_compose(const int32_t *origin_src, const unsigned *perm, long long n, int32_t *origin_dst) {
+  for (long long k = 0; k < n; ++k) origin_dst[k] = origin_src[perm[k]];
+}
+
+}
diff --git a/icebergs_amd/framework.py b/icebergs_amd/framework.py
--- a/icebergs_amd/framework.py
+++ b/icebergs_amd/framework.py
@@ -625,6 +625,11 @@
         self._check(self.lib.kid_hot_zero_mask(self.h, C.byref(m)), "kid_hot_zero_mask")
         return {name for f, name in enumerate(T.BERG_F64_NAMES) if (m.value >> f) & 1}
 
+    def cold_state(self):
+        d, m = C.c_int32(), C.c_int64()
+        self._check(self.lib.kid_cold_state(self.h, C.byref(d), C.byref(m)), "kid_cold_state")
+        return bool(d.value), m.value
+
     def profile(self, on=True):
         self._check(self.lib.kid_profile_enable(self.h, 1 if on else 0), "kid_profile_enable")
 
diff --git a/icebergs_amd/lib.py b/icebergs_amd/lib.py
--- a/icebergs_amd/lib.py
+++ b/icebergs_amd/lib.py
@@ -118,6 +118,8 @@
         lib.kid_rebin_fused_count.argtypes = [H, C.POINTER(C.c_int64)]
     if hasattr(lib, "kid_hot_zero_mask"):
         lib.kid_hot_zero_mask.argtypes = [H, C.POINTER(C.c_uint64)]
+    if hasattr(lib, "kid_cold_state"):
+        lib.kid_cold_state.argtypes = [H, C.POINTER(C.c_int32), C.POINTER(C.c_int64)]
     lib.kid_upload_bonds.argtypes = [H, C.POINTER(T.BondSoA)]
     lib.kid_download_bonds.argtypes = [H, C.POINTER(T.BondSoA)]
     lib.kid_evolve_icebergs_mts.argtypes = [H]
```

Measured after the change: 12.07 billion berg-steps/s (median of 6 runs). +2.3%, better.
